# CrossmodalGroup/DynamicVectorQuantization

Measured on AMD Instinct MI355X. Metric: images/sec (256x256) DQ-VAE train step + VQ argmin GB/s, 1/2/4/8 MI355X, higher is better.
Workload: dtype bf16

## Files before the change

### dynamicvectorquantization_amd/_lib.py

```python
from __future__ import annotations

import ctypes as C
import os

HERE = os.path.dirname(os.path.abspath(__file__))
LIB_PATH = os.path.join(HERE, "libdvq_hip.so")

F32, BF16 = 0, 1
(IMPL_AUTO, IMPL_NAIVE, IMPL_MFMA, IMPL_REGSTAGE, IMPL_HALO, IMPL_WIDE, IMPL_WIDE_PIPE, IMPL_WIDE_PIPE_4WAVE, IMPL_WIDE_PIPE_192,
 IMPL_CONV_PIPE, IMPL_8PHASE) = range(11)

vp, i64, i32, f32, sz = C.c_void_p, C.c_int64, C.c_int32, C.c_float, C.c_size_t


class ConvDesc(C.Structure):
    _fields_ = [("N", i64), ("H", i64), ("W", i64), ("Cin", i64), ("OH", i64), ("OW", i64), ("Cout", i64),
                ("KH", i32), ("KW", i32), ("stride", i32), ("pad_t", i32), ("pad_l", i32), ("upsample", i32),
                ("dtype", i32), ("impl", i32)]


class DecodeLayer(C.Structure):
    _fields_ = [(n, vp) for n in ("wq", "wk", "wv", "wo", "w1", "w2", "bq", "bk", "bv", "bo", "b1", "b2", "ln1_g", "ln1_b", "ln2_g", "ln2_b",
                                  "kcache", "vcache")]


class LinPackEntry(C.Structure):
    _fields_ = [("master", vp), ("w", vp), ("wt", vp), ("out", i64), ("in_", i64), ("out_p", i64), ("tile_begin", i64),
                ("wt_ld", i64), ("bias_src", vp), ("bias_dst", vp)]


class PackEntry(C.Structure):
    _fields_ = [("master", vp), ("w", vp), ("wt", vp), ("Cout", i64), ("Cin", i64), ("taps", i64), ("Cin_p", i64),
                ("Cout_p", i64), ("begin", i64), ("dtype", i64)]


class ScalarRecord(C.Structure):
    _fields_ = [("addr", C.c_uint64 * 64), ("code", C.c_uint8 * 64)]


class JpegInfo(C.Structure):
    _fields_ = [("width", i32), ("height", i32), ("components", i32), ("restart_interval", i32), ("h_samp", i32 * 4), ("v_samp", i32 * 4),
                ("qtab_index", i32 * 4), ("supported", i32), ("reserved", i32), ("coef_count", i64)]


(JPEG_SUPPORTED, JPEG_NOT_JPEG, JPEG_MALFORMED, JPEG_PROGRESSIVE, JPEG_ARITHMETIC, JPEG_SOF_KIND, JPEG_PRECISION, JPEG_COMPONENTS,
 JPEG_SAMPLING, JPEG_COLORSPACE, JPEG_MULTISCAN) = range(11)

SCALAR_F32, SCALAR_BF16, SCALAR_F64, SCALAR_I32, SCALAR_I64, SCALAR_IMM, SCALAR_SKIP = range(7)
SCALAR_PUSH_MAX, SCALAR_COLUMNS_MAX = 64, 256


SIGNATURES = {
    "dvq_last_error": (C.c_char_p, []),
    "dvq_last_kernel": (C.c_char_p, []),
    "dvq_version": (i32, []),
    "dvq_check_device": (i32, []),
    "dvq_set_deterministic": (i32, [i32]),
    "dvq_deterministic": (i32, []),
    "dvq_unordered_launches": (C.c_longlong, []),
    "dvq_set_fp32_split": (i32, [i32]),
    "dvq_fp32_split": (i32, []),
    "dvq_probe_mfma_rate": (i32, [i32, vp, vp, vp]),
    "dvq_vq_prep_bytes": (sz, [i64, i64]),
    "dvq_vq_prepare": (i32, [vp, i64, i64, vp, vp]),
    "dvq_vq_argmin_workspace_bytes": (sz, [i64]),
    "dvq_vq_argmin": (i32, [vp, i32, vp, vp, i64, i64, i64, vp, vp, i32, vp]),
    "dvq_vq_distances": (i32, [vp, i32, vp, i64, i64, i64, vp, vp]),
    "dvq_vq_gather_loss": (i32, [vp, i32, vp, vp, vp, i64, i64, vp, vp, vp]),
    "dvq_vq_backward": (i32, [vp, vp, i32, vp, vp, vp, vp, i64, i64, vp, vp]),
    "dvq_vq_embed": (i32, [vp, vp, i64, i64, i32, vp, vp]),
    "dvq_vq_ema_stats": (i32, [vp, i32, vp, i64, i64, i64, vp, vp]),
    "dvq_vq_ema_apply": (i32, [vp, vp, f32, f32, i64, i64, vp, vp, vp, vp, vp]),
    "dvq_patch_entropy_gate": (i32, [vp, i64, i64, i64, i32, f32, vp, vp, vp]),
    "dvq_patch_entropy_gate_range": (i32, [vp, i64, i64, i64, i32, f32, f32, f32, vp, vp, vp]),
    "dvq_gn_stats": (i32, [vp, i32, i64, i64, i64, i32, vp, vp]),
    "dvq_gn_apply": (i32, [vp, i32, i64, i64, i64, i32, f32, vp, vp, vp, i32, vp, vp, vp]),
    "dvq_gn_bwd_partial_bytes": (sz, [i64, i64, i64]),
    "dvq_gn_bwd_reduce": (i32, [vp, vp, i32, i64, i64, i64, i32, vp, vp, vp, i32, vp, vp, vp, vp, vp]),
    "dvq_gn_bwd_dx": (i32, [vp, vp, i32, i64, i64, i64, i32, vp, vp, vp, i32, vp, vp, vp, vp]),
    "dvq_conv2d_fwd": (i32, [C.POINTER(ConvDesc), vp, vp, vp, vp, vp, vp, vp, i32, i32, vp]),
    "dvq_conv3x3_fused_ok": (i32, [C.POINTER(ConvDesc)]),
    "dvq_conv3x3_subpixel_ok": (i32, [C.POINTER(ConvDesc)]),
    "dvq_split_bf16_planes": (i32, [vp, vp, vp, i64, i64, i64, vp]),
    "dvq_conv3x3_x3_ok": (i32, [C.POINTER(ConvDesc), i32]),
    "dvq_conv3x3_x3_scratch_bytes": (i64, [C.POINTER(ConvDesc), i32]),
    "dvq_conv2d_fwd_x3": (i32, [C.POINTER(ConvDesc), vp, vp, vp, vp, vp, i32, vp, i64, vp]),
    "dvq_conv2d_dgrad_x3": (i32, [C.POINTER(ConvDesc), vp, vp, vp, vp, vp, i32, vp, i64, vp]),
    "dvq_conv2d_wgrad_x3_scratch_bytes": (i64, [C.POINTER(ConvDesc)]),
    "dvq_conv2d_wgrad_oihw_x3": (i32, [C.POINTER(ConvDesc), vp, vp, i64, i64, vp, vp, i32, vp, i64, vp]),
    "dvq_gn_scale_shift": (i32, [vp, vp, vp, i64, i64, i64, i32, f32, vp, vp, vp]),
    "dvq_conv2d_dgrad": (i32, [C.POINTER(ConvDesc), vp, vp, vp, vp, vp, i32, vp]),
    "dvq_set_workspace": (i32, [vp, i64]),
    "dvq_workspace_release": (i32, [vp]),
    "dvq_cmdlist_create": (i32, [vp, C.POINTER(vp)]),
    "dvq_cmdlist_replay": (i32, [vp, vp, vp]),
    "dvq_cmdlist_info": (i32, [vp, vp]),
    "dvq_cmdlist_destroy": (i32, [vp]),
    "dvq_permute_dual": (i32, [vp, vp, i64, i32, i32, i32, i64, i64, i64, i64, i64, i64, vp, vp, vp, vp, vp, vp]),
    "dvq_permute_dual_back": (i32, [vp, vp, vp, vp, i64, i64, i64, i32, i32, i64, i64, vp, vp]),
    "dvq_avgpool_slice": (i32, [vp, i32, i64, i64, i64, i64, i32, vp, i64, i64, vp]),
    "dvq_avgpool_slice_bwd": (i32, [vp, i32, i64, i64, i64, i64, i64, i64, i32, vp, vp]),
    "dvq_silu": (i32, [vp, i32, i64, vp, vp]),
    "dvq_silu_bwd": (i32, [vp, vp, i32, i64, vp, vp]),
    "dvq_relu": (i32, [vp, i32, i64, vp, vp]),
    "dvq_relu_bwd": (i32, [vp, vp, i32, i64, vp, vp]),
    "dvq_upsample_nearest2x": (i32, [vp, i32, i64, i64, i64, i64, vp, vp]),
    "dvq_upsample_nearest2x_bwd": (i32, [vp, i32, i64, i64, i64, i64, vp, vp]),
    "dvq_grain_merge": (i32, [vp, i32, vp, vp, i32, i64, i64, i64, i64, vp, vp, vp]),
    "dvq_grain_merge_bwd": (i32, [vp, vp, i32, vp, vp, i32, i64, i64, i64, i64, vp, vp, vp]),
    "dvq_affine_channels": (i32, [vp, i32, i64, i64, vp, vp, vp, vp]),
    "dvq_axpy_dev": (i32, [vp, vp, vp, i32, i64, vp, vp]),
    "dvq_maxpool2x2": (i32, [vp, i32, i64, i64, i64, i64, vp, vp]),
    "dvq_maxpool2x2_relu_bwd": (i32, [vp, vp, vp, i32, i64, i64, i64, i64, vp, vp]),
    "dvq_lpips_head": (i32, [vp, vp, vp, i32, i64, i64, i64, vp, f32, vp, vp]),
    "dvq_lpips_head_drop": (i32, [vp, vp, vp, i32, i64, i64, i64, vp, f32, vp, f32, C.c_uint64, vp]),
    "dvq_conv2d_wgrad": (i32, [C.POINTER(ConvDesc), vp, vp, i64, i64, vp, vp, i32, vp, vp]),
    "dvq_pack_weights_multi": (i32, [vp, i64, i64, vp]),
    "dvq_linear_pack_multi": (i32, [vp, i64, i64, vp]),
    "dvq_pack_weight": (i32, [vp, i64, i64, i64, i64, i64, i64, i32, vp, vp, vp]),
    "dvq_unpack_wgrad": (i32, [vp, i64, i64, i64, i64, i64, vp, vp]),
    "dvq_nchw_to_nhwc_pad": (i32, [vp, i64, i64, i64, i64, i64, i32, vp, vp]),
    "dvq_nhwc_pad_to_nchw": (i32, [vp, i32, i64, i64, i64, i64, i64, vp, vp]),
    "dvq_gemm_nt": (i32, [vp, vp, vp, i32, i64, i64, i64, i64, i64, i64, i64, i64, i64, i64, f32, vp, i32, i32, vp]),
    "dvq_gemm_tn": (i32, [vp, vp, vp, vp, i32, i64, i64, i64, i64, i64, i64, i64, i64, i64, i64, i32, vp]),
    "dvq_softmax_rows": (i32, [vp, i32, i64, i64, f32, vp, vp]),
    "dvq_softmax_rows_bwd": (i32, [vp, vp, i32, i64, i64, f32, vp, vp]),
    "dvq_transpose": (i32, [vp, i32, i64, i64, i64, vp, vp]),
    "dvq_dual_merge": (i32, [vp, vp, vp, i32, i64, i64, i64, i64, vp, vp, vp]),
    "dvq_dual_merge_bwd": (i32, [vp, vp, i32, i64, i64, i64, i64, vp, vp, vp]),
    "dvq_add": (i32, [vp, vp, i32, i64, vp, vp]),
    "dvq_add_bias_bcast": (i32, [vp, vp, i32, i64, i64, vp, vp]),
    "dvq_channel_shift_add8": (i32, [vp, vp, i32, i64, i32, vp, vp]),
    "dvq_sum_batch": (i32, [vp, i32, i64, i64, vp, vp]),
    "dvq_sumpool2x2": (i32, [vp, i32, i64, i64, i64, i64, vp, vp]),
    "dvq_cast": (i32, [vp, i32, vp, i32, i64, vp]),
    "dvq_l1_loss": (i32, [vp, vp, i64, vp, vp, vp, vp]),
    "dvq_adam": (i32, [vp, vp, vp, vp, i64, f32, f32, f32, f32, i32, vp]),
    "dvq_adamw": (i32, [vp, vp, vp, vp, i64, f32, f32, f32, f32, f32, i32, vp]),
    "dvq_layernorm_fwd": (i32, [vp, i32, i64, i64, f32, vp, vp, vp, vp, vp]),
    "dvq_layernorm_bwd": (i32, [vp, vp, i32, i64, i64, vp, vp, vp, vp, vp, vp]),
    "dvq_layernorm_bwd_res": (i32, [vp, vp, vp, i32, i64, i64, vp, vp, vp, vp, vp, vp]),
    "dvq_layernorm_bwd_res_drop": (i32, [vp, vp, vp, i32, i64, i64, vp, vp, vp, vp, vp, vp, f32, C.c_uint64, vp]),
    "dvq_gelu": (i32, [vp, i32, i64, vp, vp]),
    "dvq_gelu_bwd": (i32, [vp, vp, i32, i64, vp, vp]),
    "dvq_softmax_causal": (i32, [vp, i32, i64, i64, i64, i64, f32, vp, vp]),
    "dvq_embed_gather": (i32, [vp, i64, vp, i32, i64, i64, i64, i64, i64, i32, vp, vp]),
    "dvq_embed_scatter_add": (i32, [vp, i64, vp, i32, i64, i64, i64, i64, i64, i64, i64, vp, vp]),
    "dvq_cross_entropy": (i32, [vp, i32, i64, i64, i64, vp, i64, vp, vp, vp, vp, vp]),
    "dvq_attn_decode": (i32, [vp, vp, vp, i32, i64, i64, i64, i64, i64, f32, vp, vp]),
    "dvq_attn_causal_ok": (i32, [i32, i64, i64, i32, i32]),
    "dvq_attn_causal_scratch_bytes": (i64, [i64, i64, i32, i32, i32]),
    "dvq_attn_causal_mask_bytes": (i64, [i64, i64, i32]),
    "dvq_attn_causal_fwd": (i32, [vp, vp, vp, i64, i32, i64, i64, i32, i32, f32, f32, C.c_uint64, vp, vp, vp, vp, vp]),
    "dvq_attn_causal_bwd": (i32, [vp, vp, vp, i64, vp, vp, vp, i32, i64, i64, i32, i32, f32, f32, C.c_uint64, vp, vp, vp, vp, vp, vp]),
    "dvq_attn_full_ok": (i32, [i32, i64, i64, i32]),
    "dvq_attn_full_fwd": (i32, [vp, vp, vp, i32, i64, i64, i32, f32, vp, vp, vp, vp]),
    "dvq_attn_full_bwd": (i32, [vp, vp, vp, vp, vp, vp, i32, i64, i64, i32, f32, vp, vp, vp, vp, vp]),
    "dvq_attn_decode_dev": (i32, [vp, vp, vp, vp, vp, i32, i64, i64, i64, vp, i64, f32, vp, vp]),
    "dvq_rows_dev": (i32, [vp, vp, i32, i64, i64, i64, vp, i32, vp]),
    "dvq_decode_stack_scratch_bytes": (sz, [i64, i64, i64]),
    "dvq_decode_stack_ok": (i32, [i64, i64, i32, i64, i64]),
    "dvq_decode_stack_status": (i32, [vp, i64, i64, i64, i32, vp]),
    "dvq_decode_stack": (i32, [vp, i32, i64, i64, i32, i64, i64, vp, C.c_float, vp, vp, i32, vp, vp]),
    "dvq_dropout": (i32, [vp, i32, i64, f32, C.c_uint64, vp, vp]),
    "dvq_dropout_add": (i32, [vp, vp, i32, i64, f32, C.c_uint64, vp, vp]),
    "dvq_fill_f32": (i32, [vp, f32, i64, vp]),
    "dvq_image_desc_bytes": (sz, []),
    "dvq_image_batch_transform": (i32, [vp, vp, vp, vp, i64, i32, i32, vp, vp]),
    "dvq_jpeg_info": (i32, [vp, sz, C.POINTER(JpegInfo)]),
    "dvq_jpeg_entropy_decode": (i32, [vp, sz, vp, i64, vp]),
    "dvq_jpeg_desc_bytes": (sz, []),
    "dvq_jpeg_batch_decode": (i32, [vp, vp, i64, vp, vp, vp]),
    "dvq_adamw_dev": (i32, [vp, vp, vp, vp, i64, vp, vp]),
    "dvq_grad_sqnorm_workspace_bytes": (sz, [i64]),
    "dvq_grad_sqnorm": (i32, [vp, i64, f32, i32, vp, sz, vp, vp]),
    "dvq_adamw_clip_dev": (i32, [vp, vp, vp, vp, i64, vp, vp, vp]),
    "dvq_ema_update": (i32, [vp, vp, i64, vp, vp, vp]),
    "dvq_swap_f32": (i32, [vp, vp, i64, vp]),
    "dvq_segment_stats_workspace_bytes": (sz, [i64, i64]),
    "dvq_segment_stats_state_bytes": (sz, [i64]),
    "dvq_segment_plan_bytes": (sz, [vp, i64, i64]),
    "dvq_segment_plan_build": (i32, [vp, i64, i64, vp, sz]),
    "dvq_segment_stats": (i32, [vp, vp, i64, vp, i64, vp, sz, vp, sz, vp, i32, vp, vp]),
    "dvq_copy_f32_armed": (i32, [vp, vp, i64, vp, vp]),
    "dvq_set_f32x8": (i32, [vp, f32, f32, f32, f32, f32, f32, f32, f32, vp]),
    "dvq_sample_rows": (i32, [vp, i64, i64, vp, vp]),
    "dvq_add_uniform": (i32, [vp, i64, f32, vp, vp]),
    "dvq_sample_constrained": (i32, [vp, i32, i64, i64, i64, f32, vp, i64, i64, i64, vp, i64, i64, i64, vp, i32, f32, i32, vp, vp, vp]),
    "dvq_sample_guided": (i32, [vp, i32, i64, i64, i64, f32, f32, vp, i64, i64, i64, vp, i64, i64, i64, vp, i32, f32, i32, vp, vp, vp]),
    "dvq_label_dropout": (i32, [vp, i64, f32, i64, C.c_uint64, vp, vp]),
    "dvq_recon_metrics_workspace_bytes": (sz, [i64, i64, i64]),
    "dvq_recon_metrics": (i32, [vp, vp, i64, i64, i64, i32, vp, vp, vp, vp, sz, vp]),
    "dvq_code_histogram": (i32, [vp, vp, i64, i64, i64, i64, i64, i64, i32, vp, vp, vp, vp]),
    "dvq_token_nll": (i32, [vp, i32, i64, i64, i64, vp, i64, vp, vp, vp]),
    "dvq_nll_segment_sums": (i32, [vp, vp, i64, i64, i64, vp, vp]),
    "dvq_tokens_pack": (i32, [vp, vp, i64, i32, i32, i64, vp, vp, vp, vp, vp]),
    "dvq_tokens_unpack": (i32, [vp, vp, i64, i32, i32, i32, i64, i64, i64, i64, i64, i64, i64, i64, vp, vp, vp, vp, vp]),
    "dvq_vq_trained_prep_bytes": (sz, [i64, i64]),
    "dvq_vq_trained_prepare": (i32, [vp, i64, i64, i32, vp, vp]),
    "dvq_vq_sample_argmax": (i32, [vp, i32, vp, vp, i64, i64, i64, i32, f32, vp, vp, vp]),
    "dvq_vq_gumbel_noise": (i32, [C.c_uint64, C.c_uint64, i64, i64, vp, vp]),
    "dvq_vq_codebook_grad": (i32, [vp, i32, vp, vp, vp, vp, i64, i64, i64, vp, vp]),
    "dvq_vq_mask_ratio": (i32, [vp, i64, vp, vp]),
    "dvq_vq_rownorm": (i32, [vp, i64, i64, vp, vp, vp]),
    "dvq_vq_ortho_scratch_bytes": (sz, []),
    "dvq_vq_ortho_sumsq": (i32, [vp, i64, f32, vp, vp, vp]),
    "dvq_vq_rownorm_bwd": (i32, [vp, vp, vp, vp, f32, i64, i64, vp, vp]),
    "dvq_imagelog_workspace_bytes": (sz, [i64]),
    "dvq_grain_overlay": (i32, [vp, vp, vp, i32, i64, i64, i64, i64, i64, C.c_uint32, C.c_uint32, f32, vp, vp, sz, vp]),
    "dvq_grain_lines": (i32, [vp, vp, i32, i64, i64, i64, i64, i64, vp]),
    "dvq_image_grid_shape": (i32, [i64, i64, i64, i64, i64, C.POINTER(i64), C.POINTER(i64)]),
    "dvq_image_grid_u8": (i32, [vp, i64, i64, i64, i64, i64, i64, i32, vp, sz, vp, sz, vp]),
    "dvq_scalar_push_state_bytes": (sz, [i64]),
    "dvq_scalar_push": (i32, [C.POINTER(ScalarRecord), i32, i32, i32, vp, vp]),
    "dvq_codebook_health": (i32, [vp, i32, i64, i64, vp, vp, vp, vp]),
    "dvq_codec_tables": (i32, [vp, i32, i64, i64, i64, vp, i64, i64, i64, vp, i64, i64, i64, vp, vp, vp]),
    "dvq_codec_record": (i32, [vp, i32, i64, i64, i64, vp, i64, i64, i64, vp, i64, i64, i64, vp, vp, vp, i64, i64, vp, vp, vp]),
    "dvq_codec_encode": (i32, [vp, i64, i64, i64, vp, vp, vp, i64, vp, vp, vp]),
    "dvq_codec_decode_step": (i32, [vp, i32, i64, i64, i64, vp, i64, i64, i64, vp, i64, i64, i64, vp, vp, vp, i64, vp, vp, vp]),
}


class DvqError(RuntimeError):
    pass


_lib = None


def load():
    global _lib
    if _lib is not None:
        return _lib
    import torch
    if not os.path.exists(LIB_PATH):
        raise DvqError(
            f"{LIB_PATH} not found. Build it with `python -m dynamicvectorquantization_amd.build` "
            "(hipcc, gfx950). There is no CPU fallback for the DQ-VAE hot path.")
    lib = C.CDLL(LIB_PATH)
    for name, (res, args) in SIGNATURES.items():
# ... 17 lines not shown
```

### dynamicvectorquantization_amd/csrc/attention.hip

```cpp
#include <type_traits>

#include "attn_common.h"

namespace {

template <int HS>
struct Geo {
    static constexpr int RROW = HS * 2 + 16;
    static constexpr int CROW = 64 + 16;
    static constexpr int RTILE = 32 * RROW;
    static constexpr int CTILE = HS * CROW;
    static constexpr int NCH = HS / 64;
};

template <int HS>
__device__ __forceinline__ void gload_rows(const bf16_t* base, int64_t rowbase, int r0, int T, int C, int tid, uint4 (&reg)[HS / 64]) {
#pragma unroll
    for (int i = 0; i < HS / 64; ++i) {
        const int id = tid + 256 * i, row = id / (HS / 8), cc = id % (HS / 8);
        reg[i] = r0 + row < T ? *reinterpret_cast<const uint4*>(base + (rowbase + r0 + row) * C + cc * 8) : make_uint4(0, 0, 0, 0);
    }
}
template <int HS>
__device__ __forceinline__ void swrite_rows(char* tile, int tid, const uint4 (&reg)[HS / 64]) {
// ... 368 lines not shown
                            if constexpr (EDGE) pr = (ok && (!diag || krow <= query)) ? pr : 0.f;
                            float gr = dp[r];
                            pk[i] = pr;
                            if constexpr (MASK) {
                                const bool keep = (mword >> (8 * g + i)) & 1u;
                                gr = keep ? gr * p.inv_keep : 0.f;
                                pk[i] = keep ? pr * p.inv_keep : 0.f;
                            } else {
                                if (p.thr != 0) {
                                    const unsigned idx = (unsigned)(((int64_t)bh * T + query) * T) + (unsigned)krow;
                                    const bool keep = dvq_hash32(idx * p.rm + p.ra) >= p.thr;
                                    gr = keep ? gr * p.inv_keep : 0.f;
                                    pk[i] = keep ? pr * p.inv_keep : 0.f;
                                }
                            }
                            ds[i] = pr * (gr - dq_[i]);
                        }
                        const unsigned p0 = pack_bf16x2(pk[0], pk[1]), p1 = pack_bf16x2(pk[2], pk[3]);
                        const unsigned d0 = pack_bf16x2(ds[0], ds[1]), d1 = pack_bf16x2(ds[2], ds[3]);
                        if (gg == 0) {
                            pf.u.x = p0; pf.u.y = p1; df.u.x = d0; df.u.y = d1;
                        } else {
                            pf.u.z = p0; pf.u.w = p1; df.u.z = d0; df.u.w = d1;
                        }
                    }
#pragma unroll
                    for (int mt = 0; mt < NM; ++mt) {
                        if constexpr (DO_DV) dv[mt] = MFMA(frag_c<HS>(dtl, l31, half, mt, s2), pf.v, dv[mt]);
                        if constexpr (DO_DK) dk[mt] = MFMA(frag_c<HS>(qtl, l31, half, mt, s2), df.v, dk[mt]);
                    }
                }
            };
            if (edge) second(std::true_type{});
            else second(std::false_type{});
        }
        if (more) {
            char* nl = smem + ((qt + 1 - kt_min) & 1) * STAGE;
            swrite_rows<HS>(nl, tid, rq);
            if constexpr (DO_DK) swrite_rows<HS>(nl + G::RTILE, tid, rd);
            if constexpr (DO_DK) swrite_cols<HS>(nl + 2 * G::RTILE, tid, rqt);
            if constexpr (DO_DV) swrite_cols<HS>(nl + 2 * G::RTILE + G::CTILE, tid, rdt);
        }
        __syncthreads();
    }
    if (kok) {
        if constexpr (DO_DV) store_ct<NM>(p.dv + (rowbase + krow) * C + h * HS, dv, half, 1.f);
        if constexpr (DO_DK) store_ct<NM>(p.dk + (rowbase + krow) * C + h * HS, dk, half, p.scale);
    }
}

template <int HS>
int launch_fwd(const AttnArgsCm& p, dim3 grid, hipStream_t stream) {
    using G = Geo<HS>;
    const int lds = 2 * (G::RTILE + G::CTILE);
    dvq_ensure_dynamic_lds((const void*)attn_fwd_kernel<HS>, lds);
    attn_fwd_kernel<HS><<<grid, dim3(256), lds, stream>>>(p);
    return 0;
}

template <int HS, bool MASKED>
int launch_bwd_m(const AttnArgsCm& p, dim3 grid, hipStream_t stream) {
    using G = Geo<HS>;
    const int lds_kv = 2 * (2 * G::RTILE + 2 * G::CTILE), lds_q = 2 * (2 * G::RTILE + G::CTILE);
    dvq_ensure_dynamic_lds((const void*)attn_bwd_dq_kernel<HS, MASKED>, lds_q);
    attn_bwd_dq_kernel<HS, MASKED><<<grid, dim3(256), lds_q, stream>>>(p);
    dvq_ensure_dynamic_lds((const void*)attn_bwd_dkv_kernel<HS, 0, MASKED>, lds_kv);
    attn_bwd_dkv_kernel<HS, 0, MASKED><<<grid, dim3(256), lds_kv, stream>>>(p);
    return 0;
}
template <int HS>
int launch_bwd(const AttnArgsCm& p, dim3 grid, hipStream_t stream) {
    if (p.thr != 0 && p.mask != nullptr) return launch_bwd_m<HS, true>(p, grid, stream);
    return launch_bwd_m<HS, false>(p, grid, stream);
}

const char* attn_refusal(int dtype, int64_t B, int64_t T, int n_head, int head_dim, int64_t ld, float p_drop, int causal) {
    if (!(dtype == DVQ_BF16 && (causal ? head_dim == 64 || head_dim == 128 : head_dim == 256)))
        return "%s: bf16 with head size 64 or 128 (causal) / 256 (full attention) only (use the GEMM path otherwise)";
    if (!(causal || T % 32 == 0)) return "%s: full attention needs T %% 32 == 0";
    if (!(B > 0 && T > 0 && T % 8 == 0 && n_head > 0 && B * n_head <= 65535 && p_drop >= 0.f && p_drop < 1.f && (causal || p_drop == 0.f)))
        return "%s: bad geometry (T %% 8 == 0, B * n_head <= 65535)";
    if (!((double)B * n_head * (double)T * (double)T < 4294967296.0))
        return "%s: B * n_head * T * T must stay below 2^32 (dropout element index)";
    if (ld != (int64_t)n_head * head_dim && head_dim != 128)
        return "%s: a row pitch other than n_head * head_dim needs head size 128 (the kernels of attention2.hip)";
    if (!(ld >= (int64_t)n_head * head_dim && ld % 8 == 0 && (double)T * (double)ld * 2.0 < 4294967296.0))
        return "%s: bad pitch (at least n_head * head_dim, a multiple of 8, T * pitch * 2 below 2^32)";
    return nullptr;
}

int fill_params(AttnArgs& p, const char* who, int dtype, int64_t B, int64_t T, int n_head, int head_dim, int64_t ld, float scale, float p_drop,
                uint64_t seed, int causal = 1) {
    if (const char* why = attn_refusal(dtype, B, T, n_head, head_dim, ld, p_drop, causal)) {
        dvq_set_error(why, who);
        return DVQ_ESHAPE;
    }
    p.causal = causal;
    p.B = (int)B; p.T = (int)T; p.nh = n_head; p.ldq = (int)ld;
    p.scale = scale;
    p.inv_keep = 1.f / (1.f - p_drop);
    p.thr = (unsigned)((double)p_drop * 4294967296.0);
    dvq_dropout_seed(seed, &p.rm, &p.ra);
    return DVQ_OK;
}

int64_t dsum_bytes(int64_t B, int64_t T, int n_head) { return ((B * n_head * T * 4 + 255) / 256) * 256; }

}

extern "C" {

int dvq_attn_causal_ok(int dtype, int64_t B, int64_t T, int n_head, int head_dim) {
    return attn_refusal(dtype, B, T, n_head, head_dim, (int64_t)n_head * head_dim, 0.f, 1) == nullptr;
}
int dvq_attn_full_ok(int dtype, int64_t B, int64_t T, int C) { return attn_refusal(dtype, B, T, 1, C, C, 0.f, 0) == nullptr; }

int64_t dvq_attn_causal_scratch_bytes(int64_t B, int64_t T, int n_head, int head_dim, int backward) {
    const int64_t copy = head_dim == 64 ? B * T * n_head * head_dim * 2 : 0;
    return backward ? 3 * copy + dsum_bytes(B, T, n_head) : copy;
}

int64_t dvq_attn_causal_mask_bytes(int64_t B, int64_t T, int n_head) {
    const int64_t nt = (T + 31) / 32;
    return B * n_head * nt * nt * 16 * 8;
}

int dvq_attn_causal_fwd(const void* q, const void* k, const void* v, int64_t ldqkv, int dtype, int64_t B, int64_t T, int n_head,
                        int head_dim, float scale, float p_drop, uint64_t seed, void* out, float* lse, void* scratch, void* drop_mask,
                        dvq_stream_t stream) {
    DVQ_REQUIRE(q && k && v && out && lse, DVQ_EINVAL, "dvq_attn_causal_fwd: null pointer");
    AttnArgsCm p{};
    int rc = fill_params(p, "dvq_attn_causal_fwd", dtype, B, T, n_head, head_dim, ldqkv, scale, p_drop, seed);
    if (rc != DVQ_OK) return rc;
    DVQ_REQUIRE(scratch || dvq_attn_causal_scratch_bytes(B, T, n_head, head_dim, 0) == 0, DVQ_EINVAL, "dvq_attn_causal_fwd: null scratch");
    p.q = (const bf16_t*)q; p.k = (const bf16_t*)k; p.v = (const bf16_t*)v;
    p.out = (bf16_t*)out; p.lse = lse;
    p.mask = (unsigned long long*)drop_mask;
    if (head_dim == 128) {
        dvq_attn2_fwd(p, (hipStream_t)stream);
        DVQ_CHECK_LAUNCH("attn_causal_fwd");
        return DVQ_OK;
    }
    p.vt = (const bf16_t*)scratch;
    rc = dvq_transpose(v, dtype, B, T, n_head * head_dim, scratch, stream);
    if (rc != DVQ_OK) return rc;
    const int nqt = (int)((T + 31) / 32);
    launch_fwd<64>(p, dim3((unsigned)((nqt + 3) / 4), (unsigned)(B * n_head)), (hipStream_t)stream);
    DVQ_CHECK_LAUNCH("attn_causal_fwd");
    return DVQ_OK;
}

int dvq_attn_causal_bwd(const void* q, const void* k, const void* v, int64_t ldqkv, const void* out, const void* dout, const float* lse,
                        int dtype, int64_t B, int64_t T, int n_head, int head_dim, float scale, float p_drop, uint64_t seed, void* dq,
                        void* dk, void* dv, void* scratch, const void* drop_mask, dvq_stream_t stream) {
    DVQ_REQUIRE(q && k && v && out && dout && lse && dq && dk && dv && scratch, DVQ_EINVAL, "dvq_attn_causal_bwd: null pointer");
    AttnArgsCm p{};
    int rc = fill_params(p, "dvq_attn_causal_bwd", dtype, B, T, n_head, head_dim, ldqkv, scale, p_drop, seed);
    if (rc != DVQ_OK) return rc;
    p.q = (const bf16_t*)q; p.k = (const bf16_t*)k; p.v = (const bf16_t*)v; p.o = (const bf16_t*)out; p.dout = (const bf16_t*)dout;
    p.dq = (bf16_t*)dq; p.dk = (bf16_t*)dk; p.dv = (bf16_t*)dv;
    p.lse = const_cast<float*>(lse);
    p.mask = (unsigned long long*)const_cast<void*>(drop_mask);
    if (head_dim == 128) {
        p.dsum = (float*)scratch;
        dvq_attn2_bwd(p, (hipStream_t)stream);
        DVQ_CHECK_LAUNCH("attn_causal_bwd");
        return DVQ_OK;
    }
    const int64_t C = n_head * head_dim, elems = B * T * C;
    bf16_t* qt = (bf16_t*)scratch;
    bf16_t* kt = qt + elems;
    bf16_t* dot = kt + elems;
    p.qt = qt; p.kt = kt; p.dot = dot;
    p.dsum = reinterpret_cast<float*>(dot + elems);
    if ((rc = dvq_transpose(q, dtype, B, T, C, qt, stream)) != DVQ_OK) return rc;
    if ((rc = dvq_transpose(k, dtype, B, T, C, kt, stream)) != DVQ_OK) return rc;
    if ((rc = dvq_transpose(dout, dtype, B, T, C, dot, stream)) != DVQ_OK) return rc;
    const int nt = (int)((T + 31) / 32);
    launch_bwd<64>(p, dim3((unsigned)((nt + 3) / 4), (unsigned)(B * n_head)), (hipStream_t)stream);
    DVQ_CHECK_LAUNCH("attn_causal_bwd");
    return DVQ_OK;
}

int dvq_attn_full_fwd(const void* q, const void* k, const void* v, int dtype, int64_t B, int64_t T, int C, float scale, void* out,
                      float* lse, void* , dvq_stream_t stream) {
    DVQ_REQUIRE(q && k && v && out && lse, DVQ_EINVAL, "dvq_attn_full_fwd: null pointer");
    AttnArgs p{};
    int rc = fill_params(p, "dvq_attn_full_fwd", dtype, B, T, 1, C, C, scale, 0.f, 0, 0);
    if (rc != DVQ_OK) return rc;
    p.q = (const bf16_t*)q; p.k = (const bf16_t*)k; p.v = (const bf16_t*)v;
    p.out = (bf16_t*)out; p.lse = lse;
    dvq_attn2_fwd(p, (hipStream_t)stream);
    DVQ_CHECK_LAUNCH("attn_full_fwd");
    return DVQ_OK;
}

int dvq_attn_full_bwd(const void* q, const void* k, const void* v, const void* out, const void* dout, const float* lse, int dtype,
                      int64_t B, int64_t T, int C, float scale, void* dq, void* dk, void* dv, void* scratch, dvq_stream_t stream) {
    DVQ_REQUIRE(q && k && v && out && dout && lse && dq && dk && dv && scratch, DVQ_EINVAL, "dvq_attn_full_bwd: null pointer");
    AttnArgs p{};
    int rc = fill_params(p, "dvq_attn_full_bwd", dtype, B, T, 1, C, C, scale, 0.f, 0, 0);
    if (rc != DVQ_OK) return rc;
    p.q = (const bf16_t*)q; p.k = (const bf16_t*)k; p.v = (const bf16_t*)v; p.o = (const bf16_t*)out; p.dout = (const bf16_t*)dout;
    p.dq = (bf16_t*)dq; p.dk = (bf16_t*)dk; p.dv = (bf16_t*)dv;
    p.lse = const_cast<float*>(lse);
    p.dsum = (float*)scratch;
    dvq_attn2_bwd(p, (hipStream_t)stream);
    DVQ_CHECK_LAUNCH("attn_full_bwd");
    return DVQ_OK;
}

}
```

### dynamicvectorquantization_amd/csrc/igemm.hip

```cpp
#include "igemm.h"

using namespace igemm;

namespace {

int conv_check(const dvq_conv_desc* d, const char* who) {
    dvq_note_kernel("");
    DVQ_REQUIRE(d != nullptr, DVQ_EINVAL, "%s: null descriptor", who);
    DVQ_REQUIRE(d->N > 0 && d->H > 0 && d->W > 0 && d->Cin > 0 && d->OH > 0 && d->OW > 0 && d->Cout > 0 && d->KH > 0 &&
                    d->KW > 0 && d->stride > 0 && d->pad_t >= 0 && d->pad_l >= 0,
                DVQ_ESHAPE, "%s: non-positive dimension", who);
    DVQ_REQUIRE(d->N * d->OH * d->OW < (1ll << 31) && d->N * d->H * d->W < (1ll << 31), DVQ_ESHAPE,
                "%s: more than 2^31 pixels", who);
    DVQ_REQUIRE(d->upsample == 0 || d->upsample == 1, DVQ_EINVAL, "%s: upsample must be 0 or 1 (2: dvq_conv2d_fwd / _dgrad only)", who);
    DVQ_REQUIRE(!d->upsample || (d->H % 2 == 0 && d->W % 2 == 0), DVQ_ESHAPE, "%s: upsample needs even H, W", who);
    DVQ_REQUIRE(d->dtype == DVQ_F32 || d->dtype == DVQ_BF16, DVQ_EINVAL, "%s: bad dtype", who);
    DVQ_REQUIRE((d->OH - 1) * d->stride - d->pad_t + d->KH - 1 < d->H + d->KH && (d->OW - 1) * d->stride - d->pad_l + d->KW - 1 < d->W + d->KW,
                DVQ_ESHAPE, "%s: inconsistent output size", who);
    return DVQ_OK;
}

}

int dvq_conv3x3_halo_try(const void* x, const void* w, const float* bias, const void* residual, void* y, int64_t N,
// ... 179 lines not shown
    }
    if (sub && residual == nullptr && gn_scale_shift == nullptr && act == DVQ_ACT_NONE) {
        const bf16_t* wsub = (const bf16_t*)w + d->Cout * 9 * d->Cin;
        const int rc = dvq_conv3x3_halo_subpixel_try(x, wsub, bias, y, d->N, d->H / 2, d->W / 2, d->Cin, d->Cout, 0, out_stats, out_groups,
                                                     (hipStream_t)stream);
        if (rc != 0) return rc < 0 ? rc : DVQ_OK;
    }
    if (halo_eligible(d)) {
        const int rc = dvq_conv3x3_halo_try(x, w, bias, residual, y, d->N, d->H, d->W, d->Cin, d->Cout, 0, d->upsample,
                                            gn_scale_shift, out_stats, out_groups, act_slope_of(act), 0, 0.f,
                                            (hipStream_t)stream);
        if (rc != 0) return rc < 0 ? rc : DVQ_OK;
    }
    DVQ_REQUIRE(gn_scale_shift == nullptr && out_stats == nullptr, DVQ_ESHAPE,
                "dvq_conv2d_fwd: fused GroupNorm needs a shape accepted by dvq_conv3x3_fused_ok");
    DVQ_REQUIRE(d->impl != DVQ_IMPL_HALO, DVQ_ESHAPE, "dvq_conv2d_fwd: shape not eligible for the halo kernel");
    NtParams p = conv_nt_params(d, MODE_FWD, x, w, y);
    p.R = residual; p.bias = bias; p.bias_mode = bias ? 1 : 0;
    p.act_slope = act_slope_of(act);
    if (d->dtype == DVQ_F32) return launch_nt<float>(p, 1, d->impl, (hipStream_t)stream);
    return launch_nt<bf16_t>(p, 1, d->impl, (hipStream_t)stream);
}

int dvq_sumpool2x2(const void* in, int dtype, int64_t N, int64_t h, int64_t w, int64_t C, void* out, dvq_stream_t stream);

int dvq_conv2d_dgrad(const dvq_conv_desc* d_in, const void* dy, const void* wt, void* dx, void* ws, const void* mask, int mask_act,
                     dvq_stream_t stream) {
    dvq_note_kernel("");
    DVQ_REQUIRE(d_in != nullptr, DVQ_EINVAL, "dvq_conv2d_dgrad: null descriptor");
    dvq_conv_desc dd = *d_in;
    const dvq_conv_desc* d = &dd;
    const int sub = conv_check_up2(&dd, "dvq_conv2d_dgrad");
    if (sub < 0) return sub;
    DVQ_REQUIRE(mask == nullptr || ((mask_act == DVQ_ACT_RELU || mask_act == DVQ_ACT_LRELU) && !d->upsample), DVQ_EINVAL,
                "dvq_conv2d_dgrad: mask needs act in {relu, lrelu} and no folded upsample");
    DVQ_REQUIRE(dy && wt && dx && (!d->upsample || ws || sub), DVQ_EINVAL, "dvq_conv2d_dgrad: null pointer");
    if (sub) {
        const bf16_t* wsub = (const bf16_t*)wt + d->Cin * 9 * d->Cout;
        const int rc = dvq_conv3x3_halo_subpixel_try(dy, wsub, nullptr, dx, d->N, d->H / 2, d->W / 2, d->Cin, d->Cout, 1, nullptr, 0,
                                                     (hipStream_t)stream);
        if (rc < 0) return rc;
        DVQ_REQUIRE(rc == 1, DVQ_ESHAPE, "dvq_conv2d_dgrad: the halo kernel refused the sub-pixel form");
        return DVQ_OK;
    }
    if (d->dtype == DVQ_BF16 && d->impl == DVQ_IMPL_AUTO && d->KH == 4 && d->KW == 4 && d->stride == 2 && d->pad_t == 1 && d->pad_l == 1 &&
        d->Cin == 8 && !d->upsample && mask == nullptr && d->H == 2 * d->OH && d->W == 2 * d->OW) {
        const int rc = dvq_tconv4x4s2_thin_try(dy, wt, dx, d->N, d->OH, d->OW, d->Cout, 4, (hipStream_t)stream);
        if (rc != 0) return rc < 0 ? rc : DVQ_OK;
    }
    if (halo_eligible(d) && d->impl == DVQ_IMPL_AUTO && d->Cout == 8 && !d->upsample && mask == nullptr) {
        const int rc = dvq_conv3x3_thin_k_try(dy, wt, nullptr, dx, d->N, d->H, d->W, d->Cin, 1, 1.f, (hipStream_t)stream);
        if (rc != 0) return rc < 0 ? rc : DVQ_OK;
    }
    if (halo_eligible(d)) {
        const int rc = dvq_conv3x3_halo_try(dy, wt, nullptr, mask, d->upsample ? ws : dx, d->N, d->H, d->W, d->Cout, d->Cin, 1,
                                            0, nullptr, nullptr, 0, 1.f, mask != nullptr, act_slope_of(mask_act),
                                            (hipStream_t)stream);
        if (rc < 0) return rc;
        if (rc == 1) return d->upsample ? dvq_sumpool2x2(ws, d->dtype, d->N, d->H / 2, d->W / 2, d->Cin, dx, stream) : DVQ_OK;
    }
    DVQ_REQUIRE(d->impl != DVQ_IMPL_HALO, DVQ_ESHAPE, "dvq_conv2d_dgrad: shape not eligible for the halo kernel");
    NtParams p = conv_nt_params(d, MODE_TCONV, dy, wt, d->upsample ? ws : dx);
    p.R = mask; p.res_mask = mask != nullptr; p.mask_slope = act_slope_of(mask_act);
    int rc = d->dtype == DVQ_F32 ? launch_nt<float>(p, 1, d->impl, (hipStream_t)stream)
                                 : launch_nt<bf16_t>(p, 1, d->impl, (hipStream_t)stream);
    if (rc) return rc;
    if (d->upsample) return dvq_sumpool2x2(ws, d->dtype, d->N, d->H / 2, d->W / 2, d->Cin, dx, stream);
    return DVQ_OK;
}

int dvq_conv2d_wgrad(const dvq_conv_desc* d, const void* x, const void* dy, int64_t cin_real, int64_t cout_real, float* grad,
                     float* dbias, int ohwi, const float* gn_scale_shift, dvq_stream_t stream) {
    if (int e = conv_check(d, "dvq_conv2d_wgrad")) return e;
    DVQ_REQUIRE(x && dy && grad && cin_real > 0 && cin_real <= d->Cin && cout_real > 0 && cout_real <= d->Cout,
                DVQ_EINVAL, "dvq_conv2d_wgrad: bad arguments");
    if (halo_eligible(d)) {
        const int rc = dvq_conv3x3_halo_wgrad_try(x, dy, grad, dbias, d->N, d->H, d->W, d->Cin, d->Cout, cin_real,
                                                  cout_real, ohwi ? 0 : 1, d->upsample, gn_scale_shift, (hipStream_t)stream);
        if (rc != 0) return rc < 0 ? rc : DVQ_OK;
    }
    DVQ_REQUIRE(gn_scale_shift == nullptr, DVQ_ESHAPE, "dvq_conv2d_wgrad: fused GroupNorm needs a shape accepted by dvq_conv3x3_fused_ok");
    DVQ_REQUIRE(d->impl != DVQ_IMPL_HALO, DVQ_ESHAPE, "dvq_conv2d_wgrad: shape not eligible for the halo kernel");
    const TnParams p = conv_tn_params(d, x, dy, cin_real, cout_real, grad, dbias, ohwi);
    if (d->dtype == DVQ_F32) return launch_tn<float>(p, 1, d->impl, (hipStream_t)stream);
    return launch_tn<bf16_t>(p, 1, d->impl, (hipStream_t)stream);
}

namespace {

__global__ __launch_bounds__(256) void split_planes_kernel(const float* __restrict__ x, bf16_t* __restrict__ hi, bf16_t* __restrict__ lo,
                                                           int64_t rows, int cin, int cout) {
    const int cpr = cout >> 3;
    const int64_t total = rows * cpr;
    for (int64_t i = (int64_t)blockIdx.x * 256 + threadIdx.x; i < total; i += (int64_t)gridDim.x * 256) {
        const int64_t r = i / cpr;
        const int c0 = (int)(i - r * cpr) << 3;
        const float* src = x + r * cin + c0;
        float4 a = make_float4(0.f, 0.f, 0.f, 0.f), b = a;
        if (c0 < cin) a = *reinterpret_cast<const float4*>(src);
        if (c0 + 4 < cin) b = *reinterpret_cast<const float4*>(src + 4);
        const float v[8] = {a.x, a.y, a.z, a.w, b.x, b.y, b.z, b.w};
        uint4 h, l;
        unsigned* hp = &h.x;
        unsigned* lp = &l.x;
#pragma unroll
        for (int e = 0; e < 4; ++e) {
            const unsigned ph = pack_bf16x2(v[2 * e], v[2 * e + 1]);
            hp[e] = ph;
            lp[e] = pack_bf16x2(v[2 * e] - __uint_as_float(ph << 16), v[2 * e + 1] - __uint_as_float(ph & 0xffff0000u));
        }
        *reinterpret_cast<uint4*>(hi + r * cout + c0) = h;
        *reinterpret_cast<uint4*>(lo + r * cout + c0) = l;
    }
}

inline int64_t pad8(int64_t c) { return (c + 7) & ~(int64_t)7; }

}

int dvq_split_bf16_planes(const float* x, void* hi, void* lo, int64_t rows, int64_t cin, int64_t cout, dvq_stream_t stream) {
    DVQ_REQUIRE(x && hi && lo, DVQ_EINVAL, "dvq_split_bf16_planes: null pointer");
    DVQ_REQUIRE(rows > 0 && cin > 0 && cin % 4 == 0 && cout % 8 == 0 && cout >= cin && cout < (1 << 20), DVQ_ESHAPE,
                "dvq_split_bf16_planes: needs cin %% 4 == 0, cout %% 8 == 0, cout >= cin");
    const int64_t total = rows * (cout / 8);
    int64_t blocks = cdiv64(total, 256);
    if (blocks > 256 * 64) blocks = 256 * 64;
    split_planes_kernel<<<dim3((unsigned)blocks), dim3(256), 0, (hipStream_t)stream>>>(x, (bf16_t*)hi, (bf16_t*)lo, rows, (int)cin, (int)cout);
    DVQ_CHECK_LAUNCH("split_planes");
    return DVQ_OK;
}

int64_t dvq_conv2d_wgrad_x3_scratch_bytes(const dvq_conv_desc* d) {
    if (d == nullptr || d->dtype != DVQ_F32) return 0;
    const int64_t xrows = d->N * (d->H >> d->upsample) * (d->W >> d->upsample), yrows = d->N * d->OH * d->OW;
    return 4 * (xrows * pad8(d->Cin) + yrows * pad8(d->Cout)) + 1024;
}

int dvq_conv2d_wgrad_oihw_x3(const dvq_conv_desc* d, const void* x, const void* dy, int64_t cin_real, int64_t cout_real,
                             float* grad_oihw, float* dbias, int ohwi, void* scratch, int64_t scratch_bytes, dvq_stream_t stream) {
    if (int e = conv_check(d, "dvq_conv2d_wgrad_oihw_x3")) return e;
    DVQ_REQUIRE(d->dtype == DVQ_F32, DVQ_EINVAL, "dvq_conv2d_wgrad_oihw_x3: fp32 operands only");
    DVQ_REQUIRE(x && dy && grad_oihw && scratch && cin_real > 0 && cin_real <= d->Cin && cout_real > 0 && cout_real <= d->Cout,
                DVQ_EINVAL, "dvq_conv2d_wgrad_oihw_x3: bad arguments");
    DVQ_REQUIRE(scratch_bytes >= dvq_conv2d_wgrad_x3_scratch_bytes(d) && ((uintptr_t)scratch & 15) == 0, DVQ_EWORKSPACE,
                "dvq_conv2d_wgrad_oihw_x3: scratch too small (dvq_conv2d_wgrad_x3_scratch_bytes) or not 16-B aligned");
    const int64_t xrows = d->N * (d->H >> d->upsample) * (d->W >> d->upsample), yrows = d->N * d->OH * d->OW;
    const int64_t c8 = pad8(d->Cin), o8 = pad8(d->Cout);
    auto up256 = [](int64_t v) { return (v + 255) & ~(int64_t)255; };
    char* base = (char*)scratch;
    char* xh = base;
    char* xl = xh + up256(xrows * c8 * 2);
    char* yh = xl + up256(xrows * c8 * 2);
    char* yl = yh + up256(yrows * o8 * 2);
    if (int e = dvq_split_bf16_planes((const float*)x, xh, xl, xrows, d->Cin, c8, stream)) return e;
    if (int e = dvq_split_bf16_planes((const float*)dy, yh, yl, yrows, d->Cout, o8, stream)) return e;
    dvq_conv_desc b = *d;
    b.dtype = DVQ_BF16;
    b.Cin = c8;
    b.Cout = o8;
    if (halo_eligible(&b) && xl == xh + xrows * c8 * 2 && yl == yh + yrows * o8 * 2) {
        const int rc = dvq_conv3x3_halo_wgrad_planes_try(xh, yh, grad_oihw, dbias, d->N, d->H, d->W, c8, o8, cin_real, cout_real, ohwi ? 0 : 1,
                                                         d->upsample, (hipStream_t)stream);
        if (rc < 0) return rc;
        if (rc == 1) return DVQ_OK;
    }
    if (int e = dvq_conv2d_wgrad(&b, xl, yh, cin_real, cout_real, grad_oihw, nullptr, ohwi, nullptr, stream)) return e;
// ... 104 lines not shown
```

### dynamicvectorquantization_amd/csrc/misc.hip

```cpp
#include <stdarg.h>

#include "dvq_common.h"
#include <stdlib.h>

static thread_local char g_err[512] = "";
thread_local const char* dvq_kernel_note = "";
void dvq_set_error(const char* fmt, ...) {
    va_list ap;
    va_start(ap, fmt);
    vsnprintf(g_err, sizeof(g_err), fmt, ap);
    va_end(ap);
}

#include <atomic>
#include <mutex>
#include <vector>
void dvq_ensure_dynamic_lds(const void* kernel, int bytes) {
    static std::mutex mu;
    static std::vector<std::pair<const void*, int>> done;
    std::lock_guard<std::mutex> lock(mu);
    for (auto& e : done)
        if (e.first == kernel && e.second >= bytes) return;
    (void)hipFuncSetAttribute(kernel, hipFuncAttributeMaxDynamicSharedMemorySize, bytes);
    done.emplace_back(kernel, bytes);
// ... 215 lines not shown

template <typename T>
__global__ __launch_bounds__(256) void sum_batch_vec_kernel(const T* __restrict__ x, int64_t batch, int64_t inner8,
                                                            float* __restrict__ out, int64_t rows_per_chunk, int cvb_log2,
                                                            float* __restrict__ part) {
    __shared__ float red[256 * 8];
    const int cvb = 1 << cvb_log2, rlanes = 256 >> cvb_log2;
    const int cv = threadIdx.x & (cvb - 1), rl = threadIdx.x >> cvb_log2;
    const int64_t c8 = (int64_t)blockIdx.x * cvb + cv;
    const int64_t b0 = (int64_t)blockIdx.y * rows_per_chunk, b1 = min(batch, b0 + rows_per_chunk);
    float acc[8] = {0.f, 0.f, 0.f, 0.f, 0.f, 0.f, 0.f, 0.f};
    if (c8 < inner8) {
        for (int64_t b = b0 + rl; b < b1; b += rlanes) {
            float v[8];
            load8(x + (b * inner8 + c8) * 8, v);
#pragma unroll
            for (int j = 0; j < 8; ++j) acc[j] += v[j];
        }
    }
#pragma unroll
    for (int j = 0; j < 8; ++j) red[(rl * cvb + cv) * 8 + j] = acc[j];
    __syncthreads();
    const int ncol = cvb * 8;
    if ((int)threadIdx.x < ncol) {
        float t = 0.f;
        for (int r = 0; r < rlanes; ++r) t += red[r * ncol + threadIdx.x];
        const int64_t col = (int64_t)blockIdx.x * ncol + threadIdx.x;
        if (col < inner8 * 8) {
            if (gridDim.y == 1) out[col] += t;
            else if (part != nullptr) part[(int64_t)blockIdx.y * inner8 * 8 + col] = t;
            else atomicAdd(&out[col], t);
        }
    }
}

template <typename T>
__global__ __launch_bounds__(256) void sumpool2x2_kernel(const T* __restrict__ in, int64_t N, int64_t h, int64_t w,
                                                         int64_t C, T* __restrict__ out) {
    const int64_t cv = C / 8;
    const int64_t total = N * h * w * cv;
    for (int64_t e = (int64_t)blockIdx.x * 256 + threadIdx.x; e < total; e += (int64_t)gridDim.x * 256) {
        const int64_t c8 = e % cv, cell = e / cv;
        const int64_t xc = cell % w, yc = (cell / w) % h, n = cell / (h * w);
        float acc[8] = {0, 0, 0, 0, 0, 0, 0, 0};
#pragma unroll
        for (int dy = 0; dy < 2; ++dy)
#pragma unroll
            for (int dx = 0; dx < 2; ++dx) {
                float v[8];
                load8(in + (((n * 2 * h + 2 * yc + dy) * 2 * w) + 2 * xc + dx) * C + c8 * 8, v);
#pragma unroll
                for (int j = 0; j < 8; ++j) acc[j] += v[j];
            }
        store8(out + cell * C + c8 * 8, acc);
    }
}

template <typename TI, typename TO>
__global__ __launch_bounds__(256) void cast_kernel(const TI* __restrict__ in, TO* __restrict__ out, int64_t n) {
    for (int64_t e = (int64_t)blockIdx.x * 256 + threadIdx.x; e < n; e += (int64_t)gridDim.x * 256)
        ElemIO<TO>::store(out + e, ElemIO<TI>::load(in + e));
}

__device__ __forceinline__ float subpixel_weight(const float* m, int64_t co, int64_t ci, int cls, int t, int64_t Cin, bool ohwi) {
    const int py = cls >> 1, px = cls & 1, a = t >> 1, b = t & 1;
    const int u0 = a ? 1 + py : 0, u1 = a ? 2 : py, v0 = b ? 1 + px : 0, v1 = b ? 2 : px;
    float s = 0.f;
    for (int u = u0; u <= u1; ++u)
        for (int v = v0; v <= v1; ++v) s += master_at(m, co, ci, u * 3 + v, Cin, 9, ohwi);
    return s;
}
__device__ __forceinline__ float subpixel_w_at(const float* m, unsigned f, unsigned Cout, unsigned Cin, bool ohwi) {
    const unsigned row = f / Cin, ci = f - row * Cin, t = row & 3, r2 = row >> 2, cls = r2 / Cout, co = r2 - cls * Cout;
    return subpixel_weight(m, co, ci, (int)cls, (int)t, Cin, ohwi);
}
__device__ __forceinline__ float subpixel_wt_at(const float* m, unsigned f, unsigned Cout, unsigned Cin, bool ohwi) {
    const unsigned row = f / Cout, co = f - row * Cout, t = row & 3, cls = (row >> 2) & 3, ci = row >> 4;
    return subpixel_weight(m, co, ci, (int)cls, (int)t, Cin, ohwi);
}

template <typename T>
__global__ __launch_bounds__(256) void pack_weight_kernel(const float* __restrict__ m, int64_t Cout, int64_t Cin,
                                                          int64_t KH, int64_t KW, int64_t Cin_p, int64_t Cout_p,
                                                          T* __restrict__ w, T* __restrict__ wt, bool ohwi, bool sub) {
    const int64_t taps = KH * KW;
    const int64_t nw = w ? Cout * taps * Cin_p : 0, nwt = wt ? Cin * taps * Cout_p : 0, nsub = sub ? 16 * Cout * Cin : 0;
    for (int64_t e = (int64_t)blockIdx.x * 256 + threadIdx.x; e < nw + nwt + 2 * nsub; e += (int64_t)gridDim.x * 256) {
        if (e >= nw + nwt) {
            const int64_t f = e - nw - nwt;
            if (f < nsub) ElemIO<T>::store(w + nw + f, subpixel_w_at(m, (unsigned)f, (unsigned)Cout, (unsigned)Cin, ohwi));
            else ElemIO<T>::store(wt + nwt + f - nsub, subpixel_wt_at(m, (unsigned)(f - nsub), (unsigned)Cout, (unsigned)Cin, ohwi));
        } else if (e < nw) {
            const int64_t ci = e % Cin_p, tap = (e / Cin_p) % taps, co = e / (Cin_p * taps);
            ElemIO<T>::store(w + e, ci < Cin ? master_at(m, co, ci, tap, Cin, taps, ohwi) : 0.f);
        } else {
            const int64_t f = e - nw;
            const int64_t co = f % Cout_p, tap = (f / Cout_p) % taps, ci = f / (Cout_p * taps);
            ElemIO<T>::store(wt + f, co < Cout ? master_at(m, co, ci, tap, Cin, taps, ohwi) : 0.f);
        }
    }
}

struct PackEntry {
    const float* master;
    void* w;
    void* wt;
    int64_t Cout, Cin, taps, Cin_p, Cout_p;
    int64_t begin;
    int64_t dtype;
};

__device__ __forceinline__ float master_at(const float* m, int64_t co, int64_t ci, int64_t tap, int64_t Cin, int64_t taps, bool ohwi) {
    return ohwi ? m[(co * taps + tap) * Cin + ci] : m[(co * Cin + ci) * taps + tap];
}

__global__ __launch_bounds__(256) void pack_weights_multi_kernel(const PackEntry* __restrict__ tab, int n, int64_t total) {
    for (int64_t e = ((int64_t)blockIdx.x * 256 + threadIdx.x) * 4; e < total; e += (int64_t)gridDim.x * 1024) {
        int lo = 0, hi = n - 1;
        while (lo < hi) {
            const int mid = (lo + hi + 1) >> 1;
            if (tab[mid].begin <= e) lo = mid; else hi = mid - 1;
        }
        const PackEntry t = tab[lo];
        const unsigned f0 = (unsigned)(e - t.begin);
        const unsigned taps = (unsigned)t.taps, Cin = (unsigned)t.Cin, Cout = (unsigned)t.Cout;
        const unsigned nw = t.w ? Cout * taps * (unsigned)t.Cin_p : 0u;
        const bool ohwi = (t.dtype >> 8) & 1;
        const unsigned nwt = t.wt ? Cin * taps * (unsigned)t.Cout_p : 0u;
        float v[4];
        void* dst;
        unsigned di;
        if (((t.dtype >> 9) & 1) && f0 >= nw + nwt) {
            const unsigned f = f0 - nw - nwt, nsub = 16u * Cout * Cin;
#pragma unroll
            for (int u = 0; u < 4; ++u)
                v[u] = f < nsub ? subpixel_w_at(t.master, f + u, Cout, Cin, ohwi) : subpixel_wt_at(t.master, f - nsub + u, Cout, Cin, ohwi);
            dst = f < nsub ? t.w : t.wt;
            di = f < nsub ? nw + f : nwt + f - nsub;
        } else if (f0 < nw) {
            const unsigned cp = (unsigned)t.Cin_p, row = f0 / cp, ci = f0 - row * cp, co = row / taps, tap = row - co * taps;
#pragma unroll
            for (int u = 0; u < 4; ++u) v[u] = ci + u < Cin ? master_at(t.master, co, ci + u, tap, Cin, taps, ohwi) : 0.f;
            dst = t.w;
            di = f0;
        } else {
            const unsigned f = f0 - nw;
            const unsigned cp = (unsigned)t.Cout_p, row = f / cp, co = f - row * cp, ci = row / taps, tap = row - ci * taps;
#pragma unroll
            for (int u = 0; u < 4; ++u) v[u] = co + u < Cout ? master_at(t.master, co + u, ci, tap, Cin, taps, ohwi) : 0.f;
            dst = t.wt;
            di = f;
        }
        if ((t.dtype & 0xff) == DVQ_F32) {
            *reinterpret_cast<float4*>(reinterpret_cast<float*>(dst) + di) = make_float4(v[0], v[1], v[2], v[3]);
        } else {
            uint2 pk;
            pk.x = (unsigned)f32_to_bf16(v[0]) | ((unsigned)f32_to_bf16(v[1]) << 16);
            pk.y = (unsigned)f32_to_bf16(v[2]) | ((unsigned)f32_to_bf16(v[3]) << 16);
            *reinterpret_cast<uint2*>(reinterpret_cast<bf16_t*>(dst) + di) = pk;
        }
    }
}

struct LinPackEntry {
    const float* master;
    bf16_t* w;
    bf16_t* wt;
    int64_t out, in, out_p;
    int64_t tile_begin;
    int64_t wt_ld;
    const float* bias_src;
    float* bias_dst;
};

__global__ __launch_bounds__(256) void linear_pack_multi_kernel(const LinPackEntry* __restrict__ tab, int n) {
    __shared__ float tile[64][65];
    int lo = 0, hi = n - 1;
    while (lo < hi) {
        const int mid = (lo + hi + 1) >> 1;
        if (tab[mid].tile_begin <= (int64_t)blockIdx.x) lo = mid; else hi = mid - 1;
    }
    const LinPackEntry t = tab[lo];
    const int tj_n = (int)((t.in + 63) >> 6);
    const int ti = (int)(((int64_t)blockIdx.x - t.tile_begin) / tj_n), tj = (int)(((int64_t)blockIdx.x - t.tile_begin) - (int64_t)ti * tj_n);
    const int r0 = ti * 64, c0 = tj * 64;
    const int q = threadIdx.x & 15, rr = threadIdx.x >> 4;
    const int64_t wt_ld = t.wt_ld != 0 ? t.wt_ld : t.out_p;
    if (t.bias_dst != nullptr && tj == 0 && threadIdx.x < 64 && r0 + (int)threadIdx.x < t.out)
        t.bias_dst[r0 + threadIdx.x] = t.bias_src[r0 + threadIdx.x];
#pragma unroll
    for (int i = 0; i < 4; ++i) {
        const int r = rr + 16 * i, row = r0 + r, col = c0 + 4 * q;
        float v[4] = {0.f, 0.f, 0.f, 0.f};
        if (row < t.out) {
            if (col + 3 < t.in && (t.in & 3) == 0 && (reinterpret_cast<uintptr_t>(t.master) & 15) == 0) {
                const float4 f = *reinterpret_cast<const float4*>(t.master + (int64_t)row * t.in + col);
                v[0] = f.x; v[1] = f.y; v[2] = f.z; v[3] = f.w;
            } else {
#pragma unroll
                for (int u = 0; u < 4; ++u) v[u] = col + u < t.in ? t.master[(int64_t)row * t.in + col + u] : 0.f;
            }
        }
#pragma unroll
        for (int u = 0; u < 4; ++u) tile[r][4 * q + u] = v[u];
        if (row < t.out_p) {
            if (col + 3 < t.in && (t.in & 3) == 0) {
                uint2 pk;
                pk.x = (unsigned)f32_to_bf16(v[0]) | ((unsigned)f32_to_bf16(v[1]) << 16);
                pk.y = (unsigned)f32_to_bf16(v[2]) | ((unsigned)f32_to_bf16(v[3]) << 16);
                *reinterpret_cast<uint2*>(t.w + (int64_t)row * t.in + col) = pk;
            } else {
#pragma unroll
                for (int u = 0; u < 4; ++u)
                    if (col + u < t.in) t.w[(int64_t)row * t.in + col + u] = f32_to_bf16(v[u]);
            }
        }
    }
    __syncthreads();
#pragma unroll
    for (int i = 0; i < 4; ++i) {
        const int c = rr + 16 * i, col = c0 + c, row = r0 + 4 * q;
        if (col < t.in && row < t.out_p) {
            uint2 pk;
            pk.x = (unsigned)f32_to_bf16(tile[4 * q][c]) | ((unsigned)f32_to_bf16(tile[4 * q + 1][c]) << 16);
            pk.y = (unsigned)f32_to_bf16(tile[4 * q + 2][c]) | ((unsigned)f32_to_bf16(tile[4 * q + 3][c]) << 16);
            *reinterpret_cast<uint2*>(t.wt + (int64_t)col * wt_ld + row) = pk;
        }
    }
}

__global__ __launch_bounds__(256) void unpack_wgrad_kernel(const float* __restrict__ dw, int64_t Cout, int64_t Cin,
                                                           int64_t taps, int64_t Cin_p, float* __restrict__ g) {
    const int64_t n = Cout * Cin * taps;
    for (int64_t e = (int64_t)blockIdx.x * 256 + threadIdx.x; e < n; e += (int64_t)gridDim.x * 256) {
// ... 548 lines not shown
                                                                                                   npix, (bf16_t*)y);
    DVQ_CHECK_LAUNCH("channel_shift_add8");
    return DVQ_OK;
}

int dvq_add_bias_bcast(const void* x, const float* bias, int dtype, int64_t batch, int64_t inner, void* y,
                       dvq_stream_t stream) {
    DVQ_REQUIRE(x && bias && y && batch > 0 && inner > 0 && inner % 8 == 0, DVQ_EINVAL, "dvq_add_bias_bcast: bad arguments");
    DVQ_DISPATCH_DTYPE(dtype, T, add_bias_bcast_kernel<T><<<dim3(nblocks(batch * inner / 8, 256)), dim3(256), 0,
                                                            (hipStream_t)stream>>>((const T*)x, bias, batch, inner / 8,
                                                                                   (T*)y););
    DVQ_CHECK_LAUNCH("add_bias_bcast");
    return DVQ_OK;
}

int dvq_sum_batch(const void* x, int dtype, int64_t batch, int64_t inner, float* out, dvq_stream_t stream) {
    DVQ_REQUIRE(x && out && batch > 0 && inner > 0, DVQ_EINVAL, "dvq_sum_batch: bad arguments");
    const bool det = dvq_deterministic() != 0;
    if (inner % 8 == 0 && batch >= 64) {
        const int64_t inner8 = inner / 8;
        int lg = 2;
        while (lg < 5 && (1 << lg) < inner8) ++lg;
        const int64_t gx = cdiv64(inner8, 1 << lg);
        int64_t chunks = gx >= 512 ? 1 : cdiv64(512, gx);
        if (chunks > cdiv64(batch, 64)) chunks = cdiv64(batch, 64);
        int64_t rpc = cdiv64(batch, chunks);
        chunks = cdiv64(batch, rpc);
        if (gx <= 65535 && chunks <= 65535) {
            float* part = nullptr;
            if (chunks > 1 && det) {
                part = (float*)dvq_det_scratch((hipStream_t)stream, chunks * inner * 4);
                if (part == nullptr) { chunks = 1; rpc = batch; }
            } else if (chunks > 1) dvq_note_unordered();
            DVQ_DISPATCH_DTYPE(dtype, T, sum_batch_vec_kernel<T><<<dim3((unsigned)gx, (unsigned)chunks), dim3(256), 0, (hipStream_t)stream>>>(
                                             (const T*)x, batch, inner8, out, rpc, lg, part););
            DVQ_CHECK_LAUNCH("sum_batch");
            if (part != nullptr) return dvq_det_fold_f32(out, part, (int)chunks, inner, inner, (hipStream_t)stream);
            return DVQ_OK;
        }
    }
    const int64_t col_blocks = cdiv64(inner, 256);
    int64_t chunks = col_blocks >= 1024 ? 1 : cdiv64(1024, col_blocks);
    if (chunks > cdiv64(batch, 16)) chunks = cdiv64(batch, 16);
    if (chunks < 1) chunks = 1;
    int64_t rpc = cdiv64(batch, chunks);
    chunks = cdiv64(batch, rpc);
    float* part = nullptr;
    if (chunks > 1 && det) {
        part = (float*)dvq_det_scratch((hipStream_t)stream, chunks * inner * 4);
        if (part == nullptr) { chunks = 1; rpc = batch; }
    } else if (chunks > 1) dvq_note_unordered();
    DVQ_DISPATCH_DTYPE(dtype, T, sum_batch_kernel<T><<<dim3((unsigned)(col_blocks < 65535 ? col_blocks : 65535), (unsigned)chunks), dim3(256), 0,
                                                      (hipStream_t)stream>>>((const T*)x, batch, inner, out, rpc, part););
    DVQ_CHECK_LAUNCH("sum_batch");
    if (part != nullptr) return dvq_det_fold_f32(out, part, (int)chunks, inner, inner, (hipStream_t)stream);
    return DVQ_OK;
}

int dvq_sumpool2x2(const void* in, int dtype, int64_t N, int64_t h, int64_t w, int64_t C, void* out,
                   dvq_stream_t stream) {
    DVQ_REQUIRE(in && out && C % 8 == 0, DVQ_EINVAL, "dvq_sumpool2x2: bad arguments");
    DVQ_DISPATCH_DTYPE(dtype, T, sumpool2x2_kernel<T><<<dim3(nblocks(N * h * w * C / 8, 256)), dim3(256), 0,
                                                        (hipStream_t)stream>>>((const T*)in, N, h, w, C, (T*)out););
    DVQ_CHECK_LAUNCH("sumpool2x2");
    return DVQ_OK;
}

int dvq_cast(const void* in, int in_dtype, void* out, int out_dtype, int64_t n, dvq_stream_t stream) {
    DVQ_REQUIRE(in && out && n > 0, DVQ_EINVAL, "dvq_cast: bad arguments");
    hipStream_t s = (hipStream_t)stream;
    dim3 grid(nblocks(n, 256)), block(256);
    if (in_dtype == DVQ_F32 && out_dtype == DVQ_BF16) cast_kernel<float, bf16_t><<<grid, block, 0, s>>>((const float*)in, (bf16_t*)out, n);
    else if (in_dtype == DVQ_BF16 && out_dtype == DVQ_F32) cast_kernel<bf16_t, float><<<grid, block, 0, s>>>((const bf16_t*)in, (float*)out, n);
    else if (in_dtype == DVQ_F32 && out_dtype == DVQ_F32) cast_kernel<float, float><<<grid, block, 0, s>>>((const float*)in, (float*)out, n);
    else if (in_dtype == DVQ_BF16 && out_dtype == DVQ_BF16) cast_kernel<bf16_t, bf16_t><<<grid, block, 0, s>>>((const bf16_t*)in, (bf16_t*)out, n);
    else {
        dvq_set_error("dvq_cast: bad dtypes");
        return DVQ_EINVAL;
    }
    DVQ_CHECK_LAUNCH("cast");
    return DVQ_OK;
}

int dvq_pack_weight(const float* master, int64_t Cout, int64_t Cin, int64_t KH, int64_t KW, int64_t Cin_p,
                    int64_t Cout_p, int dtype, void* w, void* wt, dvq_stream_t stream) {
    DVQ_REQUIRE(master && (w || wt) && Cin_p >= Cin && Cout_p >= Cout, DVQ_EINVAL, "dvq_pack_weight: bad arguments");
    const bool ohwi = (dtype >> 8) & 1;
    const bool sub = (dtype >> 9) & 1;
    DVQ_REQUIRE(!sub || (w && wt && KH == 3 && KW == 3 && Cin_p == Cin && Cout_p == Cout && 16 * Cout * Cin < (1ll << 31)), DVQ_EINVAL,
                "dvq_pack_weight: sub-pixel packs need both outputs, a 3x3 kernel and unpadded channels");
    const int64_t n = Cout * KH * KW * Cin_p + Cin * KH * KW * Cout_p + (sub ? 32 * Cout * Cin : 0);
    dtype &= 0xff;
    DVQ_DISPATCH_DTYPE(dtype, T, pack_weight_kernel<T><<<dim3(nblocks(n, 256)), dim3(256), 0, (hipStream_t)stream>>>(
                                     master, Cout, Cin, KH, KW, Cin_p, Cout_p, (T*)w, (T*)wt, ohwi, sub););
    DVQ_CHECK_LAUNCH("pack_weight");
    return DVQ_OK;
}

int dvq_pack_weights_multi(const void* table_dev, int64_t n_entries, int64_t total_work, dvq_stream_t stream) {
    DVQ_REQUIRE(table_dev && n_entries > 0 && n_entries < (1 << 30) && total_work > 0, DVQ_EINVAL, "dvq_pack_weights_multi: bad arguments");
    pack_weights_multi_kernel<<<dim3(nblocks(total_work, 1024)), dim3(256), 0, (hipStream_t)stream>>>(
        (const PackEntry*)table_dev, (int)n_entries, total_work);
    DVQ_CHECK_LAUNCH("pack_weights_multi");
    return DVQ_OK;
}

int dvq_linear_pack_multi(const void* table_dev, int64_t n_entries, int64_t total_tiles, dvq_stream_t stream) {
    DVQ_REQUIRE(table_dev && n_entries > 0 && n_entries < (1 << 30) && total_tiles > 0 && total_tiles < (1ll << 31), DVQ_EINVAL,
                "dvq_linear_pack_multi: bad arguments");
    linear_pack_multi_kernel<<<dim3((unsigned)total_tiles), dim3(256), 0, (hipStream_t)stream>>>((const LinPackEntry*)table_dev, (int)n_entries);
    DVQ_CHECK_LAUNCH("linear_pack_multi");
    return DVQ_OK;
}

int dvq_unpack_wgrad(const float* dw, int64_t Cout, int64_t Cin, int64_t KH, int64_t KW, int64_t Cin_p, float* grad,
                     dvq_stream_t stream) {
    DVQ_REQUIRE(dw && grad && Cin_p >= Cin, DVQ_EINVAL, "dvq_unpack_wgrad: bad arguments");
    unpack_wgrad_kernel<<<dim3(nblocks(Cout * Cin * KH * KW, 256)), dim3(256), 0, (hipStream_t)stream>>>(
        dw, Cout, Cin, KH * KW, Cin_p, grad);
    DVQ_CHECK_LAUNCH("unpack_wgrad");
    return DVQ_OK;
}

int dvq_nchw_to_nhwc_pad(const float* in, int64_t B, int64_t C, int64_t H, int64_t W, int64_t Cp, int dtype, void* out,
                         dvq_stream_t stream) {
    DVQ_REQUIRE(in && out && Cp >= C, DVQ_EINVAL, "dvq_nchw_to_nhwc_pad: bad arguments");
    if (C <= 4 && Cp == (dtype == DVQ_F32 ? 4 : 8)) {
        DVQ_DISPATCH_DTYPE(dtype, T, nchw_to_nhwc_px_kernel<T><<<dim3(nblocks(B * H * W, 256)), dim3(256), 0,
                                                                 (hipStream_t)stream>>>(in, B, (int)C, H * W, (T*)out););
        DVQ_CHECK_LAUNCH("nchw_to_nhwc_px");
        return DVQ_OK;
    }
    DVQ_DISPATCH_DTYPE(dtype, T, nchw_to_nhwc_pad_kernel<T><<<dim3(nblocks(B * H * W * Cp, 256)), dim3(256), 0,
                                                              (hipStream_t)stream>>>(in, B, C, H * W, Cp, (T*)out););
    DVQ_CHECK_LAUNCH("nchw_to_nhwc_pad");
    return DVQ_OK;
}

int dvq_nhwc_pad_to_nchw(const void* in, int dtype, int64_t B, int64_t C, int64_t H, int64_t W, int64_t Cp, float* out,
                         dvq_stream_t stream) {
    DVQ_REQUIRE(in && out && Cp >= C, DVQ_EINVAL, "dvq_nhwc_pad_to_nchw: bad arguments");
    DVQ_DISPATCH_DTYPE(dtype, T, nhwc_pad_to_nchw_kernel<T><<<dim3(nblocks(B * C * H * W, 256)), dim3(256), 0,
                                                              (hipStream_t)stream>>>((const T*)in, B, C, H * W, Cp, out););
    DVQ_CHECK_LAUNCH("nhwc_pad_to_nchw");
    return DVQ_OK;
}

int dvq_l1_loss(const float* x, const float* xrec, int64_t n, double* loss_sum, const float* scale_dev, float* g,
                dvq_stream_t stream) {
    DVQ_REQUIRE(x && xrec && n > 0, DVQ_EINVAL, "dvq_l1_loss: bad arguments");
    unsigned nb = nblocks(n, 1024);
    double* part = nullptr;
    if (loss_sum != nullptr && nb > 1) {
        if (dvq_deterministic() != 0) {
            part = (double*)dvq_det_scratch((hipStream_t)stream, (int64_t)nb * 8);
            if (part == nullptr) nb = 1;
        } else dvq_note_unordered();
    }
    l1_loss_kernel<<<dim3(nb), dim3(256), 0, (hipStream_t)stream>>>(x, xrec, n, loss_sum, scale_dev, g, part);
    DVQ_CHECK_LAUNCH("l1_loss");
    if (part != nullptr) return dvq_det_fold_f64(loss_sum, part, (int)nb, 1, 1, (hipStream_t)stream);
    return DVQ_OK;
}

int dvq_adam(float* p, const float* g, float* m, float* v, int64_t n, float lr, float beta1, float beta2, float eps,
             int step, dvq_stream_t stream) {
    DVQ_REQUIRE(p && g && m && v && n > 0 && step >= 1, DVQ_EINVAL, "dvq_adam: bad arguments");
    const double bc1 = 1.0 - pow((double)beta1, (double)step), bc2 = 1.0 - pow((double)beta2, (double)step);
    adam_kernel<<<dim3(nblocks(n, 1024)), dim3(256), 0, (hipStream_t)stream>>>(p, g, m, v, n, (float)(lr / bc1), beta1,
                                                                             beta2, eps, (float)(1.0 / sqrt(bc2)), 1.f);
    DVQ_CHECK_LAUNCH("adam");
    return DVQ_OK;
}

int dvq_adamw(float* p, const float* g, float* m, float* v, int64_t n, float lr, float beta1, float beta2, float eps,
              float weight_decay, int step, dvq_stream_t stream) {
    DVQ_REQUIRE(p && g && m && v && n > 0 && step >= 1 && weight_decay >= 0.f, DVQ_EINVAL, "dvq_adamw: bad arguments");
    const double bc1 = 1.0 - pow((double)beta1, (double)step), bc2 = 1.0 - pow((double)beta2, (double)step);
    adam_kernel<<<dim3(nblocks(n, 1024)), dim3(256), 0, (hipStream_t)stream>>>(p, g, m, v, n, (float)(lr / bc1), beta1,
                                                                             beta2, eps, (float)(1.0 / sqrt(bc2)),
// ... 167 lines not shown
```

### dynamicvectorquantization_amd/kernels.py

```python
from __future__ import annotations

import ctypes as C

import torch

from . import _lib
from . import runtime as rt
from ._lib import ConvDesc, check

_DT = {torch.float32: _lib.F32, torch.bfloat16: _lib.BF16}


def dt(t) -> int:
    d = t if isinstance(t, torch.dtype) else t.dtype
    if d not in _DT:
        raise TypeError(f"unsupported dtype {d}; libdvq_hip computes in float32 or bfloat16")
    return _DT[d]


def vec(dtype) -> int:
    return 4 if dtype == torch.float32 else 8


def _p(t):
# ... 298 lines not shown
              "dvq_patch_entropy_gate")
    else:
        check(lib().dvq_patch_entropy_gate_range(_p(img), b, h, w, patch, float(bins[0]), float(bins[1]), float(threshold or 0.0),
                                                 _p(ent), _p(gate), _s()), "dvq_patch_entropy_gate_range")
    return ent, gate


def gn_stats(x, groups=32):
    n, c = x.shape[0], x.shape[-1]
    hw = x.numel() // (n * c)
    stats = zeros_small((n, groups, 2), torch.float64, x.device)
    check(lib().dvq_gn_stats(_p(x), dt(x), n, hw, c, groups, _p(stats), _s()), "dvq_gn_stats")
    return stats


def gn_forward(x, gamma, beta, groups=32, eps=1e-6, silu=True, stats=None):
    n, c = x.shape[0], x.shape[-1]
    hw = x.numel() // (n * c)
    if stats is None:
        stats = gn_stats(x, groups)
    y = torch.empty_like(x)
    mr = torch.empty(n, groups, 2, dtype=torch.float32, device=x.device)
    check(lib().dvq_gn_apply(_p(x), dt(x), n, hw, c, groups, eps, _p(stats), _p(gamma), _p(beta), int(silu), _p(y), _p(mr),
                             _s()), "dvq_gn_apply")
    return y, mr


def gn_scale_shift(x, gamma, beta, groups=32, eps=1e-6, stats=None):
    n, c = x.shape[0], x.shape[-1]
    hw = x.numel() // (n * c)
    if stats is None:
        stats = gn_stats(x, groups)
    ss = torch.empty(n, c, 2, dtype=torch.float32, device=x.device)
    mr = torch.empty(n, groups, 2, dtype=torch.float32, device=x.device)
    check(lib().dvq_gn_scale_shift(_p(stats), _p(gamma), _p(beta), n, hw, c, groups, eps, _p(ss), _p(mr), _s()),
          "dvq_gn_scale_shift")
    return ss, mr


def gn_backward(x, dy, mean_rstd, gamma, beta, dgamma, dbeta, groups=32, silu=True, addend=None, fixed_stats=False):
    n, c = x.shape[0], x.shape[-1]
    hw = x.numel() // (n * c)
    red = zeros_small((n, groups, 2), torch.float64, x.device)
    part = torch.empty(lib().dvq_gn_bwd_partial_bytes(n, hw, c), dtype=torch.uint8, device=x.device)
    check(lib().dvq_gn_bwd_reduce(_p(x), _p(dy), dt(x), n, hw, c, groups, _p(mean_rstd), _p(gamma), _p(beta), int(silu),
                                  _p(red), _p(dgamma), _p(dbeta), _p(part), _s()), "dvq_gn_bwd_reduce")
    if fixed_stats:
        red.zero_()
    dx = torch.empty_like(x)
    check(lib().dvq_gn_bwd_dx(_p(x), _p(dy), dt(x), n, hw, c, groups, _p(mean_rstd), _p(gamma), _p(beta), int(silu),
                              _p(red), _p(addend), _p(dx), _s()), "dvq_gn_bwd_dx")
    return dx


def conv_desc(n, h, w, cin, cout, kh, kw, stride, pad_t, pad_l, oh, ow, upsample, dtype, impl=0) -> ConvDesc:
    return ConvDesc(n, h, w, cin, oh, ow, cout, kh, kw, stride, pad_t, pad_l, int(upsample), dt(dtype), impl)


PACK_OHWI, PACK_SUBPIXEL = 256, 512


def subpixel_pack_views(wbuf, wtbuf, cout, cin):
    n9 = cout * 9 * cin
    return (wbuf[:n9].view(cout, 3, 3, cin), wtbuf[:n9].view(cin, 3, 3, cout), wbuf[n9:].view(4, cout, 4, cin),
            wtbuf[n9:].view(cin, 4, 4, cout))


def pack_weight(master_oihw, cin_p, cout_p, dtype, want_w=True, want_wt=True, subpixel=False):
    cout, cin, kh, kw = master_oihw.shape
    dev = master_oihw.device
    if subpixel:
        w = torch.empty(25 * cout * cin, dtype=dtype, device=dev)
        wt = torch.empty(25 * cout * cin, dtype=dtype, device=dev)
        check(lib().dvq_pack_weight(_p(master_oihw), cout, cin, kh, kw, cin_p, cout_p, dt(dtype) | PACK_SUBPIXEL, _p(w), _p(wt), _s()),
              "dvq_pack_weight")
        return w, wt
    w = torch.empty(cout, kh, kw, cin_p, dtype=dtype, device=dev) if want_w else None
    wt = torch.zeros(cin_p, kh, kw, cout_p, dtype=dtype, device=dev) if want_wt else None
    check(lib().dvq_pack_weight(_p(master_oihw), cout, cin, kh, kw, cin_p, cout_p, dt(dtype), _p(w), _p(wt), _s()),
          "dvq_pack_weight")
    return w, wt


def pack_weight_into(master, cin_p, cout_p, dtype, w, wt, subpixel=False):
    cout, cin, kh, kw = master.shape
    flag = dt(dtype) | (PACK_OHWI if is_ohwi(master) else 0) | (PACK_SUBPIXEL if subpixel else 0)
    check(lib().dvq_pack_weight(_praw(master), cout, cin, kh, kw, cin_p, cout_p, flag, _p(w), _p(wt), _s()),
          "dvq_pack_weight")


def unpack_wgrad(dw, grad_oihw, cin_p):
    cout, cin, kh, kw = grad_oihw.shape
    check(lib().dvq_unpack_wgrad(_p(dw), cout, cin, kh, kw, cin_p, _p(grad_oihw), _s()), "dvq_unpack_wgrad")


def conv_fused_ok(d: ConvDesc) -> bool:
    return bool(lib().dvq_conv3x3_fused_ok(C.byref(d)))


def conv_subpixel_ok(d: ConvDesc) -> bool:
    return bool(lib().dvq_conv3x3_subpixel_ok(C.byref(d)))


def _with_subpixel(d: ConvDesc) -> ConvDesc:
    d2 = ConvDesc.from_buffer_copy(d)
    d2.upsample = 2
    return d2


ACT_NONE, ACT_SWISH, ACT_LRELU, ACT_RELU = 0, 1, 2, 3


def _x3_halo(d: ConvDesc, t, dgrad: bool) -> bool:
    return (t.dtype == torch.float32 and d.KH == 3 and d.stride == 1 and rt.switch("DVQ_X3_HALO") != "0" and
            bool(lib().dvq_fp32_split()) and bool(lib().dvq_conv3x3_x3_ok(C.byref(d), int(dgrad))))


def conv2d_fwd(d: ConvDesc, x, w, bias, residual=None, gn_ss=None, out_stats=None, out_groups=0, act=ACT_NONE, subpixel=False):
    y = torch.empty(d.N, d.OH, d.OW, d.Cout, dtype=x.dtype, device=x.device)
    fl, nb = _conv_cost(d, x.element_size())
    if gn_ss is None and out_stats is None and _x3_halo(d, x, False):
        _tag(d, "fwd x3 halo" + ("+res" if residual is not None else "") + ("+act" if act != ACT_NONE else ""))
        need = int(lib().dvq_conv3x3_x3_scratch_bytes(C.byref(d), 0))
        scratch = torch.empty(need, dtype=torch.uint8, device=x.device)
        _timed("conv_x3_halo", fl, nb, lambda: check(
            lib().dvq_conv2d_fwd_x3(C.byref(d), _p(x), _p(w), _p(bias), _p(residual), _p(y), act, _p(scratch), need, _s()),
            "dvq_conv2d_fwd_x3"))
        return y
    if _shape_tags():
        _tag(d, "fwd" + ("+res" if residual is not None else "") + ("+gn" if gn_ss is not None else "") +
             ("+st" if out_stats is not None else "") + ("+act" if act != ACT_NONE else ""))
    if out_stats is not None:
        ensure_workspace(x.device)
    dc = _with_subpixel(d) if subpixel else d
    _timed_conv(fl, nb, "dvq_conv2d_fwd", lambda:
        lib().dvq_conv2d_fwd(C.byref(dc), _p(x), _p(w), _p(bias), _p(residual), _p(y), _p(gn_ss), _p(out_stats), out_groups, act, _s()))
    return y


def conv2d_dgrad(d: ConvDesc, dy, wt, mask=None, mask_act=ACT_NONE, subpixel=False):
    sh, sw = (d.H // 2, d.W // 2) if d.upsample else (d.H, d.W)
    dx = torch.empty(d.N, sh, sw, d.Cin, dtype=dy.dtype, device=dy.device)
    ws = torch.empty(d.N, d.H, d.W, d.Cin, dtype=dy.dtype, device=dy.device) if d.upsample and not subpixel else None
    fl, nb = _conv_cost(d, dy.element_size())
    if _x3_halo(d, dy, True):
        _tag(d, "dgrad x3 halo")
        need = int(lib().dvq_conv3x3_x3_scratch_bytes(C.byref(d), 1))
        scratch = torch.empty(need, dtype=torch.uint8, device=dy.device)
        _timed("conv_x3_halo", fl, nb, lambda: check(
            lib().dvq_conv2d_dgrad_x3(C.byref(d), _p(dy), _p(wt), _p(dx), _p(ws), _p(mask), mask_act, _p(scratch), need, _s()),
            "dvq_conv2d_dgrad_x3"))
        return dx
    _tag(d, "dgrad")
    dc = _with_subpixel(d) if subpixel else d
    _timed_conv(fl, nb, "dvq_conv2d_dgrad", lambda:
        lib().dvq_conv2d_dgrad(C.byref(dc), _p(dy), _p(wt), _p(dx), _p(ws), _p(mask), mask_act, _s()))
    return dx


_workspace = {}
WORKSPACE_BYTES = 8 * (80 << 20)


def workspace_release(stream):
    if _workspace:
        lib().dvq_workspace_release(C.c_void_p(int(stream.cuda_stream)))


def copy_kernel_(dst, src):
    return torch.mul(src, 1, out=dst)


class CmdList:

    def __init__(self, graph):
        self.graph = graph
        h = C.c_void_p()
        check(lib().dvq_cmdlist_create(C.c_void_p(int(graph.raw_cuda_graph())), C.byref(h)), "dvq_cmdlist_create")
        self.handle = h
        info = (C.c_int64 * 4)()
        check(lib().dvq_cmdlist_info(h, info), "dvq_cmdlist_info")
        self.kernels, self.side_kernels, self.waits = int(info[0]), int(info[1]), int(info[2])
        self.other, self.side_open = int(info[3]) & 0xffffffff, bool(int(info[3]) >> 32)

    def replay(self, main, side):
        check(lib().dvq_cmdlist_replay(self.handle, C.c_void_p(int(main.cuda_stream)), C.c_void_p(int(side.cuda_stream))),
              "dvq_cmdlist_replay")

    def __del__(self):
        try:
            if self.handle:
                lib().dvq_cmdlist_destroy(self.handle)
                self.handle = None
        except Exception:
            pass
        self.graph = None


def ensure_workspace(device):
    device = torch.device(device)
    if _workspace.get("dev") != device:
        buf = torch.empty(WORKSPACE_BYTES, dtype=torch.uint8, device=device)
        check(lib().dvq_set_workspace(buf.data_ptr(), buf.numel()), "dvq_set_workspace")
        _workspace.update(dev=device, buf=buf)


def _wgrad_x3_planes() -> bool:
    return rt.switch("DVQ_X3_WGRAD_PLANES") != "0"


def split_bf16_planes(x2d, cout=None):
    rows, c = x2d.shape
    cout = c if cout is None else cout
    hi = torch.empty(rows, cout, dtype=torch.bfloat16, device=x2d.device)
    lo = torch.empty_like(hi)
    check(lib().dvq_split_bf16_planes(_p(x2d), _p(hi), _p(lo), rows, c, cout, _s()), "dvq_split_bf16_planes")
    return hi, lo


def conv2d_wgrad_oihw(d: ConvDesc, x, dy, cin_real, cout_real, grad_oihw, db=None, gn_ss=None):
    fl, nb = _conv_cost(d, x.element_size())
    ensure_workspace(x.device)
    if gn_ss is None and _wgrad_x3_planes() and x.dtype == torch.float32 and d.impl == 0 and bool(lib().dvq_fp32_split()):
        _tag(d, "wgrad x3 planes")
        need = int(lib().dvq_conv2d_wgrad_x3_scratch_bytes(C.byref(d)))
        scratch = torch.empty(need, dtype=torch.uint8, device=x.device)
        _timed("conv_wgrad_x3_planes", fl, nb, lambda: check(
            lib().dvq_conv2d_wgrad_oihw_x3(C.byref(d), _p(x), _p(dy), cin_real, cout_real, _praw(grad_oihw), _p(db),
                                           int(is_ohwi(grad_oihw)), _p(scratch), need, _s()), "dvq_conv2d_wgrad_oihw_x3"))
        return
    _tag(d, "wgrad")
    _timed_conv(fl, nb, "dvq_conv2d_wgrad", lambda:
        lib().dvq_conv2d_wgrad(C.byref(d), _p(x), _p(dy), cin_real, cout_real, _praw(grad_oihw), _p(db),
                               int(is_ohwi(grad_oihw)), _p(gn_ss), _s()))


def set_deterministic(on: bool):
    check(lib().dvq_set_deterministic(int(bool(on))), "dvq_set_deterministic")
    _det[0] = bool(on)


def deterministic() -> bool:
    _det[0] = bool(lib().dvq_deterministic())
    return _det[0]


def unordered_launches() -> int:
    return int(lib().dvq_unordered_launches())


def pack_weights_multi(table_dev, n_entries, total_work):
    check(lib().dvq_pack_weights_multi(_p(table_dev), n_entries, total_work, _s()), "dvq_pack_weights_multi")


def linear_pack_multi(table_dev, n_entries, total_tiles):
    check(lib().dvq_linear_pack_multi(_p(table_dev), n_entries, total_tiles, _s()), "dvq_linear_pack_multi")


_arena = {"buf": None, "off": 0}


def arena_reset(device=None, nbytes=8 << 20):
    a = _arena
    if a["buf"] is None or (device is not None and a["buf"].device != torch.device(device)):
        a["buf"] = torch.zeros(nbytes, dtype=torch.uint8, device=device or "cuda")
    else:
        a["buf"].zero_()
    a["off"] = 0


def zeros_small(shape, dtype, device):
    a = _arena
    n = 1
    for s_ in shape:
        n *= int(s_)
    nb = (n * torch.empty((), dtype=dtype).element_size() + 255) // 256 * 256
    if a["buf"] is None or a["buf"].device != torch.device(device) or a["off"] + nb > a["buf"].numel():
        return torch.zeros(shape, dtype=dtype, device=device)
    out = a["buf"][a["off"]:a["off"] + nb].view(dtype)[:n].view(shape)
    a["off"] += nb
    return out


def nchw_to_nhwc_pad(img, cp, dtype):
    b, c, h, w = img.shape
    out = torch.empty(b, h, w, cp, dtype=dtype, device=img.device)
    check(lib().dvq_nchw_to_nhwc_pad(_p(img), b, c, h, w, cp, dt(dtype), _p(out), _s()), "dvq_nchw_to_nhwc_pad")
    return out


def nhwc_pad_to_nchw(x, c):
    b, h, w, cp = x.shape
    out = torch.empty(b, c, h, w, dtype=torch.float32, device=x.device)
    check(lib().dvq_nhwc_pad_to_nchw(_p(x), dt(x), b, c, h, w, cp, _p(out), _s()), "dvq_nhwc_pad_to_nchw")
    return out


def probe_mfma_rate(random_operands=True):
    tf, mhz = C.c_float(0.0), C.c_float(0.0)
    check(lib().dvq_probe_mfma_rate(int(bool(random_operands)), C.byref(tf), C.byref(mhz), _s()), "dvq_probe_mfma_rate")
    return float(tf.value), float(mhz.value)


def gemm_nt(a, b, m, n, k, lda, ldb, ldc, batch=1, sa=0, sb=0, sc=0, alpha=1.0, bias=None, bias_mode=0, out=None,
            impl=0):
    if out is None:
        out = torch.empty(batch * m * ldc if sc == 0 else batch * sc, dtype=a.dtype, device=a.device)
    es = a.element_size()
    _timed("gemm_nt", 2 * batch * m * n * k, es * batch * (m * k + n * k + m * n), lambda: check(
        lib().dvq_gemm_nt(_p(a), _p(b), _p(out), dt(a), m, n, k, lda, ldb, ldc, batch, sa, sb, sc, alpha, _p(bias),
                          bias_mode, impl, _s()), "dvq_gemm_nt"))
    return out


def gemm_tn(a, b, mred, i, j, lda, ldb, ldc, batch=1, sa=0, sb=0, sc=0, out=None, impl=0, colsum=None):
    if out is None:
        out = torch.zeros(batch * (sc if sc else i * ldc), dtype=torch.float32, device=a.device)
    es = a.element_size()
    if a.is_cuda and es == 2 and mred >= 1024 and i >= 256 and j >= 256:
# ... 276 lines not shown

def nll_segment_sums(nll, rank, b, tp, split):
    if nll.numel() != b * tp or rank.numel() != b * tp:
        raise _lib.DvqError(f"nll_segment_sums: {nll.numel()} / {rank.numel()} rows for [{b}, {tp}]")
    out = torch.empty(b, 2, 4, dtype=torch.float64, device=nll.device)
    check(lib().dvq_nll_segment_sums(_p(nll), _p(rank), b, tp, split, _p(out), _s()), "dvq_nll_segment_sums")
    return out


def dropout_add(x, a, p, seed):
    y = torch.empty_like(x)
    check(lib().dvq_dropout_add(_p(x), _p(a), dt(x), x.numel(), float(p), int(seed) & 0xFFFFFFFFFFFFFFFF, _p(y), _s()), "dvq_dropout_add")
    return y


def dropout(x, p, seed):
    y = torch.empty_like(x)
    check(lib().dvq_dropout(_p(x), dt(x), x.numel(), float(p), int(seed) & 0xFFFFFFFFFFFFFFFF, _p(y), _s()), "dvq_dropout")
    return y


def attn_causal_ok(x, n_head, b, t):
    c = x.shape[-1]
    return (x.dtype in _DT and c % n_head == 0 and rt.switch("DVQ_NO_FUSED_ATTN") != "1" and
            bool(lib().dvq_attn_causal_ok(dt(x), b, t, n_head, c // n_head)))


def _attn_scratch(q, b, t, n_head, backward):
    nbytes = lib().dvq_attn_causal_scratch_bytes(b, t, n_head, q.shape[-1] // n_head, int(backward))
    return torch.empty(nbytes, dtype=torch.uint8, device=q.device) if nbytes else None


def _attn_pitch(a, b, c):
    s = a.stride()
    if len(s) == 2 and s[1] == 1 and b.stride() == s and c.stride() == s and a.shape == b.shape == c.shape:
        return s[0]
    if a.is_contiguous() and b.is_contiguous() and c.is_contiguous():
        return a.shape[-1]
    raise _lib.DvqError("attention operands must be contiguous, or 2-d column blocks that share one row pitch")


def attn_causal_drop_mask(q, b, t, n_head):
    return torch.empty(lib().dvq_attn_causal_mask_bytes(b, t, n_head) // 8, dtype=torch.int64, device=q.device)


def attn_causal_fwd(q, k, v, b, t, n_head, scale, p_drop=0.0, seed=0, drop_mask=None):
    ld = _attn_pitch(q, k, v)
    out = torch.empty(q.shape, dtype=q.dtype, device=q.device)
    lse = torch.empty(b, n_head, t, dtype=torch.float32, device=q.device)
    scratch = _attn_scratch(q, b, t, n_head, False)
    c = q.shape[-1]
    _timed("attn_causal_fwd", 2 * b * t * t * c, 4 * q.numel() * q.element_size(), lambda: check(
        lib().dvq_attn_causal_fwd(_praw(q), _praw(k), _praw(v), ld, dt(q), b, t, n_head, c // n_head, float(scale), float(p_drop),
                                  int(seed) & 0xFFFFFFFFFFFFFFFF, _p(out), _p(lse), _p(scratch), _p(drop_mask), _s()),
        "dvq_attn_causal_fwd"))
    return out, lse


def attn_causal_bwd(q, k, v, out, dout, lse, b, t, n_head, scale, p_drop=0.0, seed=0, drop_mask=None, grads=None):
    ld = _attn_pitch(q, k, v)
    if grads is None:
        if ld != q.shape[-1]:
            raise _lib.DvqError("attn_causal_bwd: q, k, v with a row pitch need grads laid out like them")
        grads = tuple(torch.empty_like(q) for _ in range(3))
    if _attn_pitch(*grads) != ld or grads[0].shape != q.shape:
        raise _lib.DvqError("attn_causal_bwd: grads must share the shape and row pitch of q, k, v")
    dq, dk, dv = grads
    scratch = _attn_scratch(q, b, t, n_head, True)
    c = q.shape[-1]
    _timed("attn_causal_bwd", 5 * b * t * t * c, 8 * q.numel() * q.element_size(), lambda: check(
        lib().dvq_attn_causal_bwd(_praw(q), _praw(k), _praw(v), ld, _p(out), _p(dout), _p(lse), dt(q), b, t, n_head, c // n_head,
                                  float(scale), float(p_drop), int(seed) & 0xFFFFFFFFFFFFFFFF, _praw(dq), _praw(dk), _praw(dv),
                                  _p(scratch), _p(drop_mask), _s()),
        "dvq_attn_causal_bwd"))
    return dq, dk, dv


def attn_full_ok(q, t):
    return (q.dtype in _DT and rt.switch("DVQ_NO_FUSED_ATTNBLOCK") != "1" and
            bool(lib().dvq_attn_full_ok(dt(q), q.shape[0] // max(1, t), t, q.shape[-1])))


def attn_full_fwd(q, k, v, b, t, scale):
    c = q.shape[-1]
    out = torch.empty_like(q)
    lse = torch.empty(b, t, dtype=torch.float32, device=q.device)
    scratch = _attn_scratch(q, b, t, 1, False)
    _timed("attn_full_fwd", 4 * b * t * t * c, 4 * q.numel() * q.element_size(), lambda: check(
        lib().dvq_attn_full_fwd(_p(q), _p(k), _p(v), dt(q), b, t, c, float(scale), _p(out), _p(lse), _p(scratch), _s()),
        "dvq_attn_full_fwd"))
    return out, lse


def attn_full_bwd(q, k, v, out, dout, lse, b, t, scale):
    c = q.shape[-1]
    dq, dk, dv = torch.empty_like(q), torch.empty_like(q), torch.empty_like(q)
    scratch = _attn_scratch(q, b, t, 1, True)
    _timed("attn_full_bwd", 10 * b * t * t * c, 8 * q.numel() * q.element_size(), lambda: check(
        lib().dvq_attn_full_bwd(_p(q), _p(k), _p(v), _p(out), _p(dout), _p(lse), dt(q), b, t, c, float(scale), _p(dq), _p(dk), _p(dv),
                                _p(scratch), _s()), "dvq_attn_full_bwd"))
    return dq, dk, dv


def decode_stack_scratch(b, c, f, device):
    return torch.zeros(lib().dvq_decode_stack_scratch_bytes(b, c, f), dtype=torch.uint8, device=device)


def decode_stack_ok(b, c, n_head, f, tmax) -> bool:
    return bool(lib().dvq_decode_stack_ok(b, c, n_head, f, tmax))


def decode_stack_status(scratch, b, c, f, reset=True):
    check(lib().dvq_decode_stack_status(_p(scratch), b, c, f, int(reset), _s()), "dvq_decode_stack_status")


def decode_stack(table_dev, n_layers, x, n_head, f, tmax, t_dev, eps, scratch, n_workgroups=0, table_host=None):
    b, c = x.shape
    host = None if table_host is None else C.cast(table_host, C.c_void_p)
    check(lib().dvq_decode_stack(_p(table_dev), n_layers, b, c, n_head, f, tmax, _p(t_dev), float(eps), _p(x), _p(scratch),
                                 int(n_workgroups), host, _s()), "dvq_decode_stack")
    return x


def attn_decode_dev(q, k_new, v_new, kcache, vcache, n_head, t_dev, scale):
    b, c = q.shape
    out = torch.empty_like(q)
    check(lib().dvq_attn_decode_dev(_p(q), _p(k_new), _p(v_new), _p(kcache), _p(vcache), dt(q), b, n_head, c // n_head, _p(t_dev),
                                    kcache.shape[1], scale, _p(out), _s()), "dvq_attn_decode_dev")
    return out


def rows_dev(x, hidden, t_dev, store):
    b, c = x.shape
    check(lib().dvq_rows_dev(_p(x), _p(hidden), dt(x), b, c, hidden.shape[1], _p(t_dev), int(store), _s()), "dvq_rows_dev")
    return x


def adamw_step(p, g, m, v, lr, beta1, beta2, eps, weight_decay, step):
    check(lib().dvq_adamw(_p(p), _p(g), _p(m), _p(v), p.numel(), lr, beta1, beta2, eps, weight_decay, step, _s()), "dvq_adamw")


def adamw_dev(p, g, m, v, hyper):
    check(lib().dvq_adamw_dev(_p(p), _p(g), _p(m), _p(v), p.numel(), _p(hyper), _s()), "dvq_adamw_dev")


GRAD_SQNORM_CHUNK = 32768


def grad_sqnorm_workspace_bytes(n) -> int:
    return int(lib().dvq_grad_sqnorm_workspace_bytes(int(n)))


def grad_stats_block(device):
    return torch.tensor([0, 0, 0x3F800000, 1, 0, 0, 0, 0], dtype=torch.int32, device=device)


def grad_sqnorm(g, workspace, gstat, clip=0.0, skip_nonfinite=False):
    assert g.dtype == torch.float32 and gstat.dtype == torch.int32 and gstat.numel() == 8
    check(lib().dvq_grad_sqnorm(_p(g), g.numel(), float(clip), int(bool(skip_nonfinite)), _p(workspace),
                                workspace.numel() * workspace.element_size(), _p(gstat), _s()), "dvq_grad_sqnorm")
    return gstat


def read_grad_stats(gstat) -> dict:
    h = gstat.cpu()
    return {"norm": float(h.view(torch.float64)[0]), "coef": float(h.view(torch.float32)[2]), "finite": bool(int(h[3])),
            "skipped": int(h[4])}


def adamw_clip_dev(p, g, m, v, hyper, gstat):
    check(lib().dvq_adamw_clip_dev(_p(p), _p(g), _p(m), _p(v), p.numel(), _p(hyper), _p(gstat), _s()), "dvq_adamw_clip_dev")


def ema_update(e, p, rec, gstat=None):
    assert e.dtype == torch.float32 and p.dtype == torch.float32 and rec.dtype == torch.float32 and e.numel() == p.numel()
    assert e.is_contiguous() and p.is_contiguous() and rec.numel() >= 1
    check(lib().dvq_ema_update(_p(e), _p(p), e.numel(), _p(rec), _p(gstat) if gstat is not None else None, _s()), "dvq_ema_update")
    return e


def swap_f32(a, b):
    assert a.dtype == torch.float32 and b.dtype == torch.float32 and a.numel() == b.numel()
    assert a.is_contiguous() and b.is_contiguous()
# ... 406 lines not shown
```

### dynamicvectorquantization_amd/layers.py

```python
from __future__ import annotations

import math

import torch
import torch.nn as nn

from . import kernels as K
from . import runtime as rt


class Tape:

    def __init__(self):
        self.s = {}
        self.c = {}

    def child(self, name: str) -> "Tape":
        t = self.c.get(name)
        if t is None:
            t = self.c[name] = Tape()
        return t


def _child(tape, name):
# ... 455 lines not shown
        k, s = self.kernel_size, self.stride
        if self.asym_pad:
            pt = pl = 0
            oh, ow = (h + 1 - k) // s + 1, (w + 1 - k) // s + 1
        else:
            pt = pl = self.padding
            oh, ow = (h + 2 * self.padding - k) // s + 1, (w + 2 * self.padding - k) // s + 1
        cin_p, cout_p = self._padded(x.dtype)
        assert x.shape[-1] == cin_p, f"expected {cin_p} (padded) input channels, got {x.shape[-1]}"
        return K.conv_desc(n, h, w, cin_p, cout_p, k, k, s, pt, pl, oh, ow, self.upsample, x.dtype, rt.impl())

    def _subpixel(self, d, dtype) -> bool:
        ent = self._packs.get(dtype)
        return bool(self.upsample and ent is not None and ent["sub"] and K.conv_subpixel_ok(d))

    def fused_ok(self, x) -> bool:
        return x.dtype == torch.bfloat16 and self.kernel_size == 3 and K.conv_fused_ok(self._desc(x))

    def fwd(self, x, tape, residual=None, gn_ss=None, want_stats=False, act=K.ACT_NONE):
        w, _, bias = self.packed(x.dtype)
        d = self._desc(x)
        if act != K.ACT_NONE:
            y = K.conv2d_fwd(d, x, w, bias, act=act)
            if tape is not None:
                tape.s.update(x=x, d=d, gn_ss=None)
            return y
        stats = None
        if want_stats and self.out_channels % 32 == 0 and 128 % (self.out_channels // 32) == 0 and self.fused_ok(x):
            stats = K.zeros_small((d.N, 32, 2), torch.float64, x.device)
        y = K.conv2d_fwd(d, x, w, bias, residual, gn_ss=gn_ss, out_stats=stats, out_groups=32 if stats is not None else 0,
                         subpixel=self._subpixel(d, x.dtype))
        if stats is not None:
            y._gn_stats = stats
        if tape is not None:
            tape.s.update(x=x, d=d, gn_ss=gn_ss)
        return y

    def bwd(self, dy, tape, need_dx=True, need_dw=True, mask=None, mask_act=K.ACT_NONE):
        x, d = tape.s["x"], tape.s["d"]
        side = need_dw and need_dx and rt.side_wgrad_enabled()
        dx = None
        if side:
            _, wt, _ = self.packed(x.dtype)
            dx = K.conv2d_dgrad(d, dy, wt, mask=mask, mask_act=mask_act, subpixel=self._subpixel(d, x.dtype))
        if need_dw:
            db = _grad_buf(self.bias) if self.bias is not None else None
            gw, gss = _grad_buf(self.weight), tape.s.get("gn_ss")
            if side:
                rt.run_on_side(lambda: K.conv2d_wgrad_oihw(d, x, dy, self.in_channels, self.out_channels, gw, db, gn_ss=gss), x, dy)
            else:
                K.conv2d_wgrad_oihw(d, x, dy, self.in_channels, self.out_channels, gw, db, gn_ss=gss)
        if not need_dx:
            return None
        if dx is not None:
            return dx
        _, wt, _ = self.packed(x.dtype)
        return K.conv2d_dgrad(d, dy, wt, mask=mask, mask_act=mask_act, subpixel=self._subpixel(d, x.dtype))


def conv1x1_bwd_accumulate(conv, dy, tape, acc):
    x, d = tape.s["x"], tape.s["d"]
    ok = (conv.kernel_size == 1 and conv.stride == 1 and conv.padding == 0 and not conv.upsample and not conv.asym_pad and
          dy.dtype == torch.bfloat16 and rt.impl() == 0 and acc is not None and d.Cin == conv.in_channels and d.Cout == conv.out_channels)
    if not ok:
        dx = conv.bwd(dy, tape)
        return dx if acc is None else K.add(dx, acc)
    _, wt, _ = conv.packed(x.dtype)
    dt_ = K.conv_desc(d.N, d.H, d.W, d.Cout, d.Cin, 1, 1, 1, 0, 0, d.H, d.W, False, dy.dtype, d.impl)
    dx = K.conv2d_fwd(dt_, dy, wt, None, acc)
    db = _grad_buf(conv.bias) if conv.bias is not None else None
    gw = _grad_buf(conv.weight)
    if rt.side_wgrad_enabled():
        rt.run_on_side(lambda: K.conv2d_wgrad_oihw(d, x, dy, conv.in_channels, conv.out_channels, gw, db), x, dy)
    else:
        K.conv2d_wgrad_oihw(d, x, dy, conv.in_channels, conv.out_channels, gw, db)
    return dx


class _PackRegistry:

    def __init__(self):
        self.items = {}
        self.tables = {}
        self.retired = []

    def register(self, mod, dtype):
        import weakref
        key = (dtype, mod.weight.device)
        self.items.setdefault(key, []).append(weakref.ref(mod))
        for k in [k for k in self.tables if k[:2] == key]:
            self.retired.append(self.tables.pop(k))

    def repack(self, dtype, device, group=0):
        import ctypes
        from ._lib import PackEntry
        key = (dtype, device)
        mods = [m for m in (r() for r in self.items.get(key, [])) if m is not None and dtype in m._packs and
                getattr(m.weight, "_dvq_group", 0) == group]
        key = (dtype, device, group)
        live = [m for m in mods if m._packs[dtype]["master"] == m.weight.data_ptr() and m._packs[dtype]["w"].device == device]
        if len(live) < 2:
            return
        sig = tuple((m.weight.data_ptr(), m._packs[dtype]["w"].data_ptr(), m.weight.stride()) for m in live)
        tab = self.tables.get(key)
        if tab is None or tab["sig"] != sig:
            arr = (PackEntry * len(live))()
            begin = 0
            for i, m in enumerate(live):
                e = m._packs[dtype]
                k2 = m.kernel_size * m.kernel_size
                arr[i] = PackEntry(m.weight.data_ptr(), e["w"].data_ptr(), e["wt"].data_ptr(), m.out_channels, m.in_channels,
                                   k2, e["cin_p"], e["cout_p"], begin, K.dt(dtype) | (K.PACK_OHWI if K.is_ohwi(m.weight) else 0) |
                                   (K.PACK_SUBPIXEL if e["sub"] else 0))
                begin += m.out_channels * k2 * e["cin_p"] + m.in_channels * k2 * e["cout_p"]
                if e["sub"]:
                    begin += 32 * m.out_channels * m.in_channels
            raw = torch.frombuffer(bytearray(bytes(arr)), dtype=torch.uint8).to(device)
            tab = {"sig": sig, "table": raw, "n": len(live), "total": begin}
            if key in self.tables:
                self.retired.append(self.tables[key])
            self.tables[key] = tab
        K.pack_weights_multi(tab["table"], tab["n"], tab["total"])
        for m in live:
            m._packs[dtype]["epoch"] = m._pack_key()


PACKS = _PackRegistry()


class Upsample(HipModule):

    def __init__(self, in_channels, with_conv):
        super().__init__()
        self.with_conv = with_conv
        if with_conv:
            self.conv = Conv2d(in_channels, in_channels, 3, stride=1, padding=1, upsample=True)

    def fwd(self, x, tape):
        if not self.with_conv:
            return K.upsample_nearest2x(x)
        return self.conv.fwd(x, _child(tape, "conv"), want_stats=True)

    def bwd(self, dy, tape):
        if not self.with_conv:
            return K.upsample_nearest2x_bwd(dy)
        return self.conv.bwd(dy, tape.child("conv"))


class Downsample(HipModule):

    def __init__(self, in_channels, with_conv):
        super().__init__()
        self.with_conv = with_conv
        if with_conv:
            self.conv = Conv2d(in_channels, in_channels, 3, stride=2, padding=0, asym_pad=True)

    def fwd(self, x, tape):
        if not self.with_conv:
            n, h, w, c = x.shape
            y = torch.empty(n, h // 2, w // 2, c, dtype=x.dtype, device=x.device)
            K.avgpool_slice(x[:, : 2 * (h // 2), : 2 * (w // 2)].contiguous() if (h | w) & 1 else x, 2, y, 0)
            if tape is not None:
                tape.s["in_hw"] = (h, w)
            return y
        return self.conv.fwd(x, _child(tape, "conv"))

    def bwd(self, dy, tape):
        if not self.with_conv:
            dx = K.avgpool_slice_bwd(dy, 0, dy.shape[-1], 2)
            h, w = tape.s["in_hw"]
            if (h | w) & 1:
                dx = torch.nn.functional.pad(dx, (0, 0, 0, w - dx.shape[2], 0, h - dx.shape[1]))
            return dx
        return self.conv.bwd(dy, tape.child("conv"))


def norm_swish_conv(norm, conv, x, tape, nname, cname, residual=None):
    if (rt.fuse_gn_prologue() or tape is None) and conv.fused_ok(x):
        ss = norm.prep(x, _child(tape, nname))
        return conv.fwd(x, _child(tape, cname), residual=residual, gn_ss=ss, want_stats=True)
    a = norm.fwd(x, _child(tape, nname), silu=True)
    return conv.fwd(a, _child(tape, cname), residual=residual, want_stats=True)


class ResnetBlock(HipModule):

    def __init__(self, *, in_channels, out_channels=None, conv_shortcut=False, dropout=0.0, temb_channels=512):
        super().__init__()
        out_channels = in_channels if out_channels is None else out_channels
        if temb_channels > 0:
            raise NotImplementedError("temb_channels > 0 is unused by the DQ-VAE (temb is None)")
        self.dropout = nn.Dropout(dropout)
        self.in_channels, self.out_channels = in_channels, out_channels
        self.use_conv_shortcut = conv_shortcut
        self.norm1 = Normalize(in_channels)
        self.conv1 = Conv2d(in_channels, out_channels, 3, 1, 1)
        self.norm2 = Normalize(out_channels)
        self.conv2 = Conv2d(out_channels, out_channels, 3, 1, 1)
        if in_channels != out_channels:
            if conv_shortcut:
                self.conv_shortcut = Conv2d(in_channels, out_channels, 3, 1, 1)
            else:
                self.nin_shortcut = Conv2d(in_channels, out_channels, 1, 1, 0)

    def _shortcut(self):
        return self.conv_shortcut if self.use_conv_shortcut else self.nin_shortcut

    def forward(self, x, temb=None, **kw):
        assert temb is None
        return super().forward(x, **kw)

    def fwd(self, x, tape, temb=None):
        h1 = norm_swish_conv(self.norm1, self.conv1, x, tape, "norm1", "conv1")
        sc = self._shortcut().fwd(x, _child(tape, "nin")) if self.in_channels != self.out_channels else x
        if self.training and self.dropout.p > 0.0:
            a = self.norm2.fwd(h1, _child(tape, "norm2"), silu=True)
            seed = rt.next_dropout_seed()
            if tape is not None:
                tape.s["drop"] = (float(self.dropout.p), seed)
            a = K.dropout(a, float(self.dropout.p), seed)
            return self.conv2.fwd(a, _child(tape, "conv2"), residual=sc, want_stats=True)
        return norm_swish_conv(self.norm2, self.conv2, h1, tape, "norm2", "conv2", residual=sc)

    def bwd(self, dy, tape):
        d = self.conv2.bwd(dy, tape.child("conv2"))
        if "drop" in tape.s:
            d = K.dropout(d, *tape.s["drop"])
        d = self.norm2.bwd(d, tape.child("norm2"))
        d = self.conv1.bwd(d, tape.child("conv1"))
        sc = self._shortcut().bwd(dy, tape.child("nin")) if self.in_channels != self.out_channels else dy
        return self.norm1.bwd(d, tape.child("norm1"), addend=sc)


class AttnBlock(HipModule):

    def __init__(self, in_channels):
        super().__init__()
        self.in_channels = in_channels
        self.norm = Normalize(in_channels)
        self.q = Conv2d(in_channels, in_channels, 1)
        self.k = Conv2d(in_channels, in_channels, 1)
        self.v = Conv2d(in_channels, in_channels, 1)
        self.proj_out = Conv2d(in_channels, in_channels, 1)

    def fwd(self, x, tape):
        b, h, w, c = x.shape
        n = h * w
        hn = self.norm.fwd(x, _child(tape, "norm"), silu=False)
        q = self.q.fwd(hn, _child(tape, "q"))
        k = self.k.fwd(hn, _child(tape, "k"))
        v = self.v.fwd(hn, _child(tape, "v"))
        impl = rt.impl()
        if impl == 0 and K.attn_full_ok(q.view(b * n, c), n):
            o, lse = K.attn_full_fwd(q.view(b * n, c), k.view(b * n, c), v.view(b * n, c), b, n, float(int(c) ** (-0.5)))
            y = self.proj_out.fwd(o.view(b, h, w, c), _child(tape, "proj"), residual=x)
            if tape is not None:
                tape.s.update(q=q, k=k, v=v, o=o, lse=lse, p=None, shape=(b, h, w, c))
            return y
        s = K.gemm_nt(q, k, n, n, c, c, c, n, batch=b, sa=n * c, sb=n * c, sc=n * n, impl=impl)
        p = K.softmax_rows(s, b * n, n, float(int(c) ** (-0.5)))
        vt = K.transpose(v, b, n, c)
        o = K.gemm_nt(p, vt, n, c, n, n, n, c, batch=b, sa=n * n, sb=c * n, sc=n * c, impl=impl)
        o = o.view(b, h, w, c)
        y = self.proj_out.fwd(o, _child(tape, "proj"), residual=x)
        if tape is not None:
            tape.s.update(q=q, k=k, v=v, p=p, shape=(b, h, w, c))
        return y

    def bwd(self, dy, tape):
        st = tape.s
        b, h, w, c = st["shape"]
        n = h * w
        q, k, v, p = st["q"], st["k"], st["v"], st["p"]
        impl = rt.impl()
        do = self.proj_out.bwd(dy, tape.child("proj"))
        if p is None:
            dq, dk, dv = K.attn_full_bwd(q.view(b * n, c), k.view(b * n, c), v.view(b * n, c), st["o"], do.view(b * n, c), st["lse"],
                                         b, n, float(int(c) ** (-0.5)))
            dh = self.q.bwd(dq.view(b, h, w, c), tape.child("q"))
            dh = conv1x1_bwd_accumulate(self.k, dk.view(b, h, w, c), tape.child("k"), dh)
            dh = conv1x1_bwd_accumulate(self.v, dv.view(b, h, w, c), tape.child("v"), dh)
            return self.norm.bwd(dh, tape.child("norm"), addend=dy)
        dp = K.gemm_nt(do, v, n, n, c, c, c, n, batch=b, sa=n * c, sb=n * c, sc=n * n, impl=impl)
        dv32 = K.gemm_tn(p, do, n, n, c, n, c, c, batch=b, sa=n * n, sb=n * c, sc=n * c, impl=impl)
        ds = K.softmax_rows_bwd(p, dp, b * n, n, float(int(c) ** (-0.5)))
        kt = K.transpose(k, b, n, c)
        dq = K.gemm_nt(ds, kt, n, c, n, n, n, c, batch=b, sa=n * n, sb=c * n, sc=n * c, impl=impl)
        dk32 = K.gemm_tn(ds, q, n, n, c, n, c, c, batch=b, sa=n * n, sb=n * c, sc=n * c, impl=impl)
        dt_ = q.dtype
        dq = dq.view(b, h, w, c)
        dk = K.cast(dk32.view(b, h, w, c), dt_)
        dv = K.cast(dv32.view(b, h, w, c), dt_)
        dh = self.q.bwd(dq, tape.child("q"))
        dh = conv1x1_bwd_accumulate(self.k, dk, tape.child("k"), dh)
        dh = conv1x1_bwd_accumulate(self.v, dv, tape.child("v"), dh)
        return self.norm.bwd(dh, tape.child("norm"), addend=dy)
```

### dynamicvectorquantization_amd/runtime.py

```python
from __future__ import annotations

import contextlib
import os

import torch

from . import _lib

_compute_dtype = torch.float32
_weights_epoch = 0
IMPL_CHOICES = (_lib.IMPL_AUTO, _lib.IMPL_NAIVE, _lib.IMPL_MFMA, _lib.IMPL_REGSTAGE, _lib.IMPL_HALO, _lib.IMPL_CONV_PIPE)
_impl = _lib.IMPL_AUTO


SWITCHES = {
    "DVQ_FUSE_GN": ("0", "1: GroupNorm+swish inside the consuming 3x3 conv on taped forwards too"),
    "DVQ_X3_HALO": ("1", "0: fp32x3 3x3 forward / input gradient on the fp32 kernel that splits at every fragment read"),
    "DVQ_X3_WGRAD_PLANES": ("1", "0: fp32x3 weight gradients on the fp32 kernel that splits at every fragment read"),
    "DVQ_NO_FUSED_ATTN": ("0", "1: causal attention as per-head GEMMs + softmax instead of the fused kernels"),
    "DVQ_NO_FUSED_ATTNBLOCK": ("0", "1: AttnBlock on GEMMs + softmax (stores the [B,N,N] probabilities)"),
    "DVQ_QKV_FUSED": ("1", "0: key / query / value as three Linear layers instead of one GEMM"),
    "DVQ_FUSE_DROP_BWD": ("1", "0: stand-alone dropout passes in the StackGPT backward"),
    "DVQ_GEN_SIDE": ("1", "0: generator loss with the PatchGAN branch on the main stream"),
    "DVQ_LOSS_PREFETCH": ("1", "0: target-only loss work inside the loss call instead of beside the autoencoder's forward"),
    "DVQ_SIDE_WGRAD": ("1", "0: weight gradients on the main stream"),
    "DVQ_STEP_GRAPH": ("1", "0: every training step eager, nothing recorded"),
    "DVQ_DECODE_GRAPH": ("1", "0: single-row sampler steps eager, nothing recorded"),
    "DVQ_DECODE_STACK": ("1", "0: a sampler token step as per-kernel launches instead of the persistent kernel"),
    "DVQ_DECODE_WGS": ("0", "n: workgroups of the persistent token-step kernel (0: the library chooses)"),
    "DVQ_PROFILE_SHAPES": ("0", "1: the profiler splits the conv families by call geometry"),
    "DVQ_GRAPH_DEBUG": ("0", "1: print the library calls of every recorded segment, synchronise after every replayed item"),
    "DVQ_GRAPH_BREAK_EVERY": ("0", "n: with DVQ_GRAPH_DEBUG=1, cut a recorded segment every n library calls"),
    "DVQ_FORCE_DP": ("0", "1: the data-parallel path in a one-rank group"),
    "DVQ_DP_CHECK_EVERY": ("0", "k: assert that the replicas are equal every k steps"),
    "DVQ_DP_NO_HOOK": ("0", "1: no all-reduce launch from inside the backward"),
    "DVQ_DP_NOOP_COLLECTIVES": ("0", "1: exchange points without the RCCL calls"),
}


def switch(name: str) -> str:
    return os.environ.get(name, SWITCHES[name][0])


def force_dp() -> bool:
    return switch("DVQ_FORCE_DP") == "1"


def compute_dtype() -> torch.dtype:
    return _compute_dtype


_fp32_split = None


def fp32_split() -> bool:
    from . import _lib
    return bool(_lib.load().dvq_fp32_split())


def set_fp32_split(on):
    global _fp32_split
    from . import _lib
    _fp32_split = None if on is None else bool(on)
    if on is not None:
        _lib.check(_lib.load().dvq_set_fp32_split(int(bool(on))), "dvq_set_fp32_split")


def set_compute_dtype(dtype):
    global _compute_dtype
    if isinstance(dtype, str):
        if dtype in ("fp32x3", "float32x3"):
            set_fp32_split(True)
            dtype = torch.float32
        else:
            if dtype in ("fp32", "float32") and _fp32_split:
                set_fp32_split(False)
            dtype = {"fp32": torch.float32, "float32": torch.float32, "bf16": torch.bfloat16, "bfloat16": torch.bfloat16}[dtype]
    assert dtype in (torch.float32, torch.bfloat16)
    _compute_dtype = dtype


@contextlib.contextmanager
def compute_dtype_ctx(dtype):
    global _fp32_split
    old, old_flag = _compute_dtype, _fp32_split
    old_lib = fp32_split() if isinstance(dtype, str) and dtype.startswith(("fp32", "float32")) else None
    set_compute_dtype(dtype)
    try:
        yield
    finally:
        set_compute_dtype(old)
        if old_lib is not None and fp32_split() != old_lib:
            set_fp32_split(old_lib)
        _fp32_split = old_flag


def weights_epoch() -> int:
    return _weights_epoch


def bump_weights_epoch():
    global _weights_epoch
    _weights_epoch += 1

# ... 288 lines not shown
```

### include/dvq_hip.h

```cpp
#ifndef DVQ_HIP_H
#define DVQ_HIP_H

#include <stddef.h>
#include <stdint.h>

#ifdef __cplusplus
extern "C" {
#endif

typedef void* dvq_stream_t;
typedef void* dvq_cmdlist_t;

enum { DVQ_F32 = 0, DVQ_BF16 = 1 };
enum { DVQ_OK = 0, DVQ_EINVAL = -1, DVQ_ESHAPE = -2, DVQ_EARCH = -3, DVQ_ELAUNCH = -4, DVQ_EWORKSPACE = -5 };

const char* dvq_last_error(void);
const char* dvq_last_kernel(void);
int dvq_version(void);
int dvq_check_device(void);
int dvq_set_deterministic(int on);
int dvq_deterministic(void);
long long dvq_unordered_launches(void);
int dvq_set_fp32_split(int on);
int dvq_fp32_split(void);
// ... 11 lines not shown

int dvq_vq_gather_loss(const void* x, int dtype, const float* codebook, const int64_t* idx, const float* mask,
                       int64_t N, int64_t D, void* x_q, double* loss_sum, dvq_stream_t stream);
int dvq_vq_backward(const void* g_xq, const void* x, int dtype, const float* codebook, const int64_t* idx,
                    const float* mask, const float* coef_dev, int64_t N, int64_t D, void* dx, dvq_stream_t stream);
int dvq_vq_embed(const float* codebook, const int64_t* idx, int64_t N, int64_t D, int out_dtype, void* out,
                 dvq_stream_t stream);

int dvq_vq_ema_stats(const void* x, int dtype, const int64_t* idx, int64_t N, int64_t K, int64_t D, float* stats,
                     dvq_stream_t stream);
int dvq_vq_ema_apply(const float* stats, const float* restart_rows, float decay, float eps, int64_t K, int64_t D,
                     float* cluster_size_ema, float* embed_ema, float* weight, float* scratch_sum,
                     dvq_stream_t stream);

int dvq_patch_entropy_gate(const float* img, int64_t B, int64_t H, int64_t W, int patch, float threshold,
                           float* entropy, int64_t* gate, dvq_stream_t stream);
int dvq_patch_entropy_gate_range(const float* img, int64_t B, int64_t H, int64_t W, int patch, float bin_lo, float bin_hi,
                                 float threshold, float* entropy, int64_t* gate, dvq_stream_t stream);

int dvq_gn_stats(const void* x, int dtype, int64_t N, int64_t HW, int64_t C, int G, double* stats,
                 dvq_stream_t stream);
int dvq_gn_apply(const void* x, int dtype, int64_t N, int64_t HW, int64_t C, int G, float eps, const double* stats,
                 const float* gamma, const float* beta, int silu, void* y, float* mean_rstd, dvq_stream_t stream);
size_t dvq_gn_bwd_partial_bytes(int64_t N, int64_t HW, int64_t C);
int dvq_gn_bwd_reduce(const void* x, const void* dy, int dtype, int64_t N, int64_t HW, int64_t C, int G,
                      const float* mean_rstd, const float* gamma, const float* beta, int silu, double* red,
                      float* dgamma, float* dbeta, float* partials, dvq_stream_t stream);
int dvq_gn_bwd_dx(const void* x, const void* dy, int dtype, int64_t N, int64_t HW, int64_t C, int G,
                  const float* mean_rstd, const float* gamma, const float* beta, int silu, const double* red,
                  const void* addend, void* dx, dvq_stream_t stream);

enum {
    DVQ_IMPL_AUTO = 0,
    DVQ_IMPL_NAIVE = 1,
    DVQ_IMPL_MFMA = 2,
    DVQ_IMPL_REGSTAGE = 3,
    DVQ_IMPL_HALO = 4,
    DVQ_IMPL_WIDE = 5,
    DVQ_IMPL_WIDE_PIPE = 6,
    DVQ_IMPL_WIDE_PIPE_4WAVE = 7,
    DVQ_IMPL_WIDE_PIPE_192 = 8,
    DVQ_IMPL_CONV_PIPE = 9,
    DVQ_IMPL_8PHASE = 10
};

typedef struct dvq_conv_desc {
    int64_t N;
    int64_t H, W;
    int64_t Cin;
    int64_t OH, OW;
    int64_t Cout;
    int32_t KH, KW;
    int32_t stride;
    int32_t pad_t, pad_l;
    int32_t upsample;
    int32_t dtype;
    int32_t impl;
} dvq_conv_desc;

enum { DVQ_ACT_NONE = 0, DVQ_ACT_SWISH = 1, DVQ_ACT_LRELU = 2, DVQ_ACT_RELU = 3 };

int dvq_conv3x3_fused_ok(const dvq_conv_desc* d);
int dvq_conv3x3_subpixel_ok(const dvq_conv_desc* d);
int dvq_conv2d_fwd(const dvq_conv_desc* d, const void* x, const void* w, const float* bias, const void* residual, void* y,
                   const float* gn_scale_shift, double* out_stats, int out_groups, int act, dvq_stream_t stream);
int dvq_split_bf16_planes(const float* x, void* hi, void* lo, int64_t rows, int64_t cin, int64_t cout, dvq_stream_t stream);
int64_t dvq_conv2d_wgrad_x3_scratch_bytes(const dvq_conv_desc* d);
int dvq_conv2d_wgrad_oihw_x3(const dvq_conv_desc* d, const void* x, const void* dy, int64_t cin_real, int64_t cout_real,
                             float* grad_oihw, float* dbias, int ohwi, void* scratch, int64_t scratch_bytes, dvq_stream_t stream);
int dvq_conv3x3_x3_ok(const dvq_conv_desc* d, int dgrad);
int64_t dvq_conv3x3_x3_scratch_bytes(const dvq_conv_desc* d, int dgrad);
int dvq_conv2d_fwd_x3(const dvq_conv_desc* d, const void* x, const void* w, const float* bias, const void* residual, void* y, int act,
                      void* scratch, int64_t scratch_bytes, dvq_stream_t stream);
int dvq_conv2d_dgrad_x3(const dvq_conv_desc* d, const void* dy, const void* wt, void* dx, void* ws, const void* mask, int mask_act,
                        void* scratch, int64_t scratch_bytes, dvq_stream_t stream);
int dvq_gn_scale_shift(const double* stats, const float* gamma, const float* beta, int64_t N, int64_t HW, int64_t C, int G,
                       float eps, float* scale_shift, float* mean_rstd, dvq_stream_t stream);

int dvq_conv2d_dgrad(const dvq_conv_desc* d, const void* dy, const void* wt, void* dx, void* ws, const void* mask, int mask_act,
                     dvq_stream_t stream);

int dvq_conv2d_wgrad(const dvq_conv_desc* d, const void* x, const void* dy, int64_t cin_real, int64_t cout_real, float* grad,
                     float* dbias, int ohwi, const float* gn_scale_shift, dvq_stream_t stream);

int dvq_pack_weights_multi(const void* table_dev, int64_t n_entries, int64_t total_work, dvq_stream_t stream);
int dvq_linear_pack_multi(const void* table_dev, int64_t n_entries, int64_t total_tiles, dvq_stream_t stream);

int dvq_pack_weight(const float* master, int64_t Cout, int64_t Cin, int64_t KH, int64_t KW, int64_t Cin_p,
                    int64_t Cout_p, int dtype, void* w, void* wt, dvq_stream_t stream);
int dvq_unpack_wgrad(const float* dw, int64_t Cout, int64_t Cin, int64_t KH, int64_t KW, int64_t Cin_p, float* grad,
                     dvq_stream_t stream);
int dvq_nchw_to_nhwc_pad(const float* in, int64_t B, int64_t C, int64_t H, int64_t W, int64_t Cp, int dtype, void* out,
                         dvq_stream_t stream);
int dvq_nhwc_pad_to_nchw(const void* in, int dtype, int64_t B, int64_t C, int64_t H, int64_t W, int64_t Cp, float* out,
                         dvq_stream_t stream);

int dvq_gemm_nt(const void* A, const void* B, void* C, int dtype, int64_t M, int64_t N, int64_t K, int64_t lda,
                int64_t ldb, int64_t ldc, int64_t batch, int64_t sA, int64_t sB, int64_t sC, float alpha,
                const float* bias, int bias_mode, int impl, dvq_stream_t stream);
int dvq_gemm_tn(const void* A, const void* B, float* C, float* colsum, int dtype, int64_t Mred, int64_t I, int64_t J, int64_t lda,
                int64_t ldb, int64_t ldc, int64_t batch, int64_t sA, int64_t sB, int64_t sC, int impl, dvq_stream_t stream);

int dvq_set_workspace(void* ptr, int64_t bytes);
int dvq_workspace_release(dvq_stream_t stream);

int dvq_cmdlist_create(void* hip_graph, dvq_cmdlist_t* out);
int dvq_cmdlist_replay(dvq_cmdlist_t list, dvq_stream_t main_stream, dvq_stream_t side_stream);
int dvq_cmdlist_info(dvq_cmdlist_t list, int64_t* info4);
int dvq_cmdlist_destroy(dvq_cmdlist_t list);

int dvq_affine_channels(const void* x, int dtype, int64_t n, int64_t C, const float* a, const float* b, void* y,
                        dvq_stream_t stream);
int dvq_axpy_dev(const void* a, const void* b, const float* scale_dev, int dtype, int64_t n, void* y, dvq_stream_t stream);
int dvq_maxpool2x2(const void* x, int dtype, int64_t N, int64_t h, int64_t w, int64_t C, void* y, dvq_stream_t stream);
int dvq_maxpool2x2_relu_bwd(const void* a, const void* dpool, const void* dtap, int dtype, int64_t N, int64_t h, int64_t w,
                            int64_t C, void* dz, dvq_stream_t stream);
int dvq_lpips_head(const void* f0, const void* f1, const float* lin, int dtype, int64_t N, int64_t HW, int64_t C, float* val,
                   float gscale, void* df1, dvq_stream_t stream);
int dvq_lpips_head_drop(const void* f0, const void* f1, const float* lin, int dtype, int64_t N, int64_t HW, int64_t C, float* val,
                        float gscale, void* df1, float p_drop, uint64_t seed, dvq_stream_t stream);

int dvq_avgpool_slice(const void* x, int dtype, int64_t N, int64_t h, int64_t w, int64_t C, int k, void* y, int64_t ldy,
                      int64_t coff, dvq_stream_t stream);
int dvq_avgpool_slice_bwd(const void* dy, int dtype, int64_t ldy, int64_t coff, int64_t N, int64_t h, int64_t w, int64_t C,
                          int k, void* dx, dvq_stream_t stream);
int dvq_silu(const void* x, int dtype, int64_t n, void* y, dvq_stream_t stream);
int dvq_silu_bwd(const void* x, const void* dy, int dtype, int64_t n, void* dx, dvq_stream_t stream);
int dvq_relu(const void* x, int dtype, int64_t n, void* y, dvq_stream_t stream);
int dvq_relu_bwd(const void* x, const void* dy, int dtype, int64_t n, void* dx, dvq_stream_t stream);
int dvq_upsample_nearest2x(const void* x, int dtype, int64_t N, int64_t h, int64_t w, int64_t C, void* y, dvq_stream_t stream);
int dvq_upsample_nearest2x_bwd(const void* dy, int dtype, int64_t N, int64_t h, int64_t w, int64_t C, void* dx, dvq_stream_t stream);
int dvq_grain_merge(const void* const* heads, int S, const int64_t* idx, const float* scale, int dtype, int64_t N, int64_t hc,
                    int64_t wc, int64_t C, void* out, float* mask, dvq_stream_t stream);
int dvq_grain_merge_bwd(const void* g_out, const void* const* heads, int S, const int64_t* idx, const float* scale, int dtype,
                        int64_t N, int64_t hc, int64_t wc, int64_t C, void* const* dheads, float* dscale, dvq_stream_t stream);

int dvq_permute_dual(const int64_t* indices, const int64_t* grain, int64_t B, int hw1, int hw2, int order, int64_t content_pad,
                     int64_t content_eos, int64_t cpos_pad, int64_t cpos_eos, int64_t fpos_pad, int64_t fpos_eos,
                     int64_t* coarse_content, int64_t* coarse_position, int64_t* fine_content, int64_t* fine_position,
                     int* counts, dvq_stream_t stream);
int dvq_permute_dual_back(const int64_t* coarse_content, const int64_t* fine_content, const int64_t* coarse_position,
                          const int64_t* fine_position, int64_t B, int64_t Lc, int64_t Lf, int hw1, int hw2, int64_t cpos_eos,
                          int64_t fpos_eos, int64_t* out, dvq_stream_t stream);

int dvq_softmax_rows(const void* s, int dtype, int64_t rows, int64_t L, float scale, void* p, dvq_stream_t stream);
int dvq_softmax_rows_bwd(const void* p, const void* dp, int dtype, int64_t rows, int64_t L, float scale, void* ds,
                         dvq_stream_t stream);
int dvq_transpose(const void* in, int dtype, int64_t batch, int64_t R, int64_t C, void* out, dvq_stream_t stream);

int dvq_dual_merge(const void* h_fine, const void* h_coarse, const int64_t* grain, int dtype, int64_t B, int64_t h,
                   int64_t w, int64_t C, void* h_dual, float* mask, dvq_stream_t stream);
int dvq_dual_merge_bwd(const void* g_dual, const int64_t* grain, int dtype, int64_t B, int64_t h, int64_t w,
                       int64_t C, void* g_fine, void* g_coarse, dvq_stream_t stream);
int dvq_add(const void* a, const void* b, int dtype, int64_t n, void* y, dvq_stream_t stream);
int dvq_add_bias_bcast(const void* x, const float* bias, int dtype, int64_t batch, int64_t inner, void* y,
                       dvq_stream_t stream);
int dvq_channel_shift_add8(const void* a, const void* b, int dtype, int64_t npix, int shift, void* y, dvq_stream_t stream);
int dvq_sum_batch(const void* x, int dtype, int64_t batch, int64_t inner, float* out, dvq_stream_t stream);
int dvq_sumpool2x2(const void* in, int dtype, int64_t N, int64_t h, int64_t w, int64_t C, void* out,
                   dvq_stream_t stream);
int dvq_cast(const void* in, int in_dtype, void* out, int out_dtype, int64_t n, dvq_stream_t stream);
int dvq_l1_loss(const float* x, const float* xrec, int64_t n, double* loss_sum, const float* scale_dev, float* g,
                dvq_stream_t stream);
int dvq_adam(float* p, const float* g, float* m, float* v, int64_t n, float lr, float beta1, float beta2, float eps,
             int step, dvq_stream_t stream);
int dvq_adamw(float* p, const float* g, float* m, float* v, int64_t n, float lr, float beta1, float beta2, float eps,
              float weight_decay, int step, dvq_stream_t stream);

int dvq_layernorm_fwd(const void* x, int dtype, int64_t rows, int64_t C, float eps, const float* gamma, const float* beta, void* y,
                      float* mean_rstd, dvq_stream_t stream);
int dvq_layernorm_bwd(const void* x, const void* dy, int dtype, int64_t rows, int64_t C, const float* mean_rstd, const float* gamma,
                      void* dx, float* dgamma, float* dbeta, dvq_stream_t stream);
int dvq_layernorm_bwd_res(const void* x, const void* dy, const void* dres, int dtype, int64_t rows, int64_t C, const float* mean_rstd,
                          const float* gamma, void* dx, float* dgamma, float* dbeta, dvq_stream_t stream);
int dvq_layernorm_bwd_res_drop(const void* x, const void* dy, const void* dres, int dtype, int64_t rows, int64_t C, const float* mean_rstd,
                               const float* gamma, void* dx, float* dgamma, float* dbeta, void* dx_drop, float p_drop, uint64_t seed,
                               dvq_stream_t stream);
int dvq_gelu(const void* x, int dtype, int64_t n, void* y, dvq_stream_t stream);
int dvq_gelu_bwd(const void* x, const void* dy, int dtype, int64_t n, void* dx, dvq_stream_t stream);
int dvq_softmax_causal(const void* s, int dtype, int64_t rows, int64_t L, int64_t Tq, int64_t offset, float scale, void* p,
                       dvq_stream_t stream);
int dvq_embed_gather(const int64_t* idx, int64_t idx_bstride, const float* table, int dtype, int64_t B, int64_t len, int64_t Ttot,
                     int64_t t0, int64_t C, int accumulate, void* out, dvq_stream_t stream);
int dvq_embed_scatter_add(const int64_t* idx, int64_t idx_bstride, const void* dout, int dtype, int64_t B, int64_t len, int64_t Ttot,
                          int64_t t0, int64_t C, int64_t padding_idx, int64_t V, float* dtable, dvq_stream_t stream);
int dvq_cross_entropy(const void* logits, int dtype, int64_t rows, int64_t V, int64_t ldl, const int64_t* target, int64_t ignore_index,
                      float* loss_sum, float* count, const float* gscale_dev, void* dlogits, dvq_stream_t stream);
int dvq_sample_constrained(const void* logits, int dtype, int64_t B, int64_t V, int64_t ldl, float temperature,
                           const int64_t* forbid_idx, int64_t n_forbid, int64_t forbid_ld, int64_t forbid_from,
                           const int64_t* forbid_codes4, int64_t keep_code, int64_t late_forbid_code, int64_t pad_code,
                           const float* finished, int top_k, float top_p, int sample, uint64_t* state, int64_t* out,
                           dvq_stream_t stream);
int dvq_sample_guided(const void* logits, int dtype, int64_t B, int64_t V, int64_t ldl, float guidance, float temperature,
                      const int64_t* forbid_idx, int64_t n_forbid, int64_t forbid_ld, int64_t forbid_from,
                      const int64_t* forbid_codes4, int64_t keep_code, int64_t late_forbid_code, int64_t pad_code,
                      const float* finished, int top_k, float top_p, int sample, uint64_t* state, int64_t* out,
                      dvq_stream_t stream);
int dvq_attn_causal_ok(int dtype, int64_t B, int64_t T, int n_head, int head_dim);
int64_t dvq_attn_causal_scratch_bytes(int64_t B, int64_t T, int n_head, int head_dim, int backward);
int64_t dvq_attn_causal_mask_bytes(int64_t B, int64_t T, int n_head);
int dvq_attn_causal_fwd(const void* q, const void* k, const void* v, int64_t ldqkv, int dtype, int64_t B, int64_t T, int n_head,
                        int head_dim, float scale, float p_drop, uint64_t seed, void* out, float* lse, void* scratch, void* drop_mask,
                        dvq_stream_t stream);
int dvq_attn_causal_bwd(const void* q, const void* k, const void* v, int64_t ldqkv, const void* out, const void* dout, const float* lse,
                        int dtype, int64_t B, int64_t T, int n_head, int head_dim, float scale, float p_drop, uint64_t seed, void* dq,
                        void* dk, void* dv, void* scratch, const void* drop_mask, dvq_stream_t stream);
int dvq_attn_full_ok(int dtype, int64_t B, int64_t T, int C);
int dvq_attn_full_fwd(const void* q, const void* k, const void* v, int dtype, int64_t B, int64_t T, int C, float scale, void* out,
                      float* lse, void* scratch, dvq_stream_t stream);
int dvq_attn_full_bwd(const void* q, const void* k, const void* v, const void* out, const void* dout, const float* lse, int dtype,
                      int64_t B, int64_t T, int C, float scale, void* dq, void* dk, void* dv, void* scratch, dvq_stream_t stream);
int dvq_attn_decode(const void* q, const void* kcache, const void* vcache, int dtype, int64_t B, int64_t n_head, int64_t head_size,
                    int64_t T, int64_t Tmax, float scale, void* out, dvq_stream_t stream);
int dvq_attn_decode_dev(const void* q, const void* k_new, const void* v_new, void* kcache, void* vcache, int dtype, int64_t B,
                        int64_t n_head, int64_t head_size, const int64_t* t_dev, int64_t Tmax, float scale, void* out,
                        dvq_stream_t stream);
int dvq_rows_dev(void* x, void* hidden, int dtype, int64_t B, int64_t C, int64_t Tmax, const int64_t* t_dev, int store,
                 dvq_stream_t stream);

typedef struct dvq_decode_layer {
    const void *wq, *wk, *wv, *wo, *w1, *w2;
    const float *bq, *bk, *bv, *bo, *b1, *b2;
    const float *ln1_g, *ln1_b, *ln2_g, *ln2_b;
    void *kcache, *vcache;
} dvq_decode_layer;
size_t dvq_decode_stack_scratch_bytes(int64_t B, int64_t C, int64_t F);
int dvq_decode_stack_ok(int64_t B, int64_t C, int n_head, int64_t F, int64_t Tmax);
int dvq_decode_stack_status(const void* scratch, int64_t B, int64_t C, int64_t F, int reset, dvq_stream_t stream);
int dvq_decode_stack(const void* layers_dev, int n_layers, int64_t B, int64_t C, int n_head, int64_t F, int64_t Tmax, const int64_t* t_dev,
                     float eps, void* x, void* scratch, int n_workgroups, const void* layers_host, dvq_stream_t stream);
int dvq_dropout(const void* x, int dtype, int64_t n, float p, uint64_t seed, void* y, dvq_stream_t stream);
int dvq_dropout_add(const void* x, const void* a, int dtype, int64_t n, float p, uint64_t seed, void* y, dvq_stream_t stream);
int dvq_label_dropout(const int64_t* labels, int64_t B, float p, int64_t null_label, uint64_t seed, int64_t* out, dvq_stream_t stream);

int dvq_adamw_dev(float* p, const float* g, float* m, float* v, int64_t n, const float* hyper, dvq_stream_t stream);
size_t dvq_grad_sqnorm_workspace_bytes(int64_t n);
int dvq_grad_sqnorm(const float* g, int64_t n, float clip, int skip_nonfinite, void* workspace, size_t workspace_bytes,
                    void* gstat, dvq_stream_t stream);
int dvq_adamw_clip_dev(float* p, const float* g, float* m, float* v, int64_t n, const float* hyper, const void* gstat,
                       dvq_stream_t stream);
int dvq_ema_update(float* e, const float* p, int64_t n, const float* rec, const void* gstat, dvq_stream_t stream);
int dvq_swap_f32(float* a, float* b, int64_t n, dvq_stream_t stream);
size_t dvq_segment_stats_workspace_bytes(int64_t n, int64_t S);
size_t dvq_segment_stats_state_bytes(int64_t S);
size_t dvq_segment_plan_bytes(const int64_t* offsets, int64_t S, int64_t n);
int dvq_segment_plan_build(const int64_t* offsets, int64_t S, int64_t n, void* plan_host, size_t plan_host_bytes);
int dvq_segment_stats(const float* a, const float* b, int64_t n, const int64_t* offsets, int64_t S, const void* plan_dev,
                      size_t plan_bytes, void* workspace, size_t workspace_bytes, void* state, int sticky, const int* armed,
                      dvq_stream_t stream);
int dvq_copy_f32_armed(float* dst, const float* src, int64_t n, const int* armed, dvq_stream_t stream);
int dvq_set_f32x8(float* dst, float v0, float v1, float v2, float v3, float v4, float v5, float v6, float v7,
                  dvq_stream_t stream);
enum { DVQ_SCALAR_F32 = 0, DVQ_SCALAR_BF16 = 1, DVQ_SCALAR_F64 = 2, DVQ_SCALAR_I32 = 3, DVQ_SCALAR_I64 = 4, DVQ_SCALAR_IMM = 5,
       DVQ_SCALAR_SKIP = 6  };
enum { DVQ_SCALAR_PUSH_MAX = 64, DVQ_SCALAR_COLUMNS_MAX = 256 };
typedef struct {
    uint64_t addr[64];
    uint8_t code[64];
} dvq_scalar_record;
size_t dvq_scalar_push_state_bytes(int64_t columns);
int dvq_scalar_push(const dvq_scalar_record* rec, int32_t count, int32_t col0, int32_t columns, void* state, dvq_stream_t stream);
int dvq_codebook_health(const void* counts, int counts_type, int64_t K, int64_t stride, float* out3, double* out3_f64, double* total,
                        dvq_stream_t stream);
int dvq_sample_rows(int64_t* out, int64_t k, int64_t n, uint64_t* state, dvq_stream_t stream);
int dvq_add_uniform(float* x, int64_t n, float scale, uint64_t* state, dvq_stream_t stream);

int dvq_fill_f32(float* p, float v, int64_t n, dvq_stream_t stream);

size_t dvq_image_desc_bytes(void);
int dvq_image_batch_transform(const uint8_t* src, const void* desc, const int32_t* tables, uint8_t* tmp, int64_t B, int S,
                              int max_rows, float* out, dvq_stream_t stream);

enum {
    DVQ_JPEG_SUPPORTED = 0,
    DVQ_JPEG_NOT_JPEG = 1,
    DVQ_JPEG_MALFORMED = 2,
    DVQ_JPEG_PROGRESSIVE = 3,
    DVQ_JPEG_ARITHMETIC = 4,
    DVQ_JPEG_SOF_KIND = 5,
    DVQ_JPEG_PRECISION = 6,
    DVQ_JPEG_COMPONENTS = 7,
    DVQ_JPEG_SAMPLING = 8,
    DVQ_JPEG_COLORSPACE = 9,
    DVQ_JPEG_MULTISCAN = 10
};
typedef struct dvq_jpeg_info_t {
    int32_t width, height, components, restart_interval;
    int32_t h_samp[4], v_samp[4], qtab_index[4];
    int32_t supported;
    int32_t reserved;
    int64_t coef_count;
} dvq_jpeg_info_t;
int dvq_jpeg_info(const uint8_t* data, size_t n, dvq_jpeg_info_t* info);
int dvq_jpeg_entropy_decode(const uint8_t* data, size_t n, int16_t* coef, int64_t coef_capacity, uint16_t* qtab);
// ... 63 lines not shown
```

Baseline: 448.1.

## Fuse AttnBlock q/k/v 1x1 convolutions into one packed GEMM with pitched attention

AttnBlock now packs the q, k and v 1x1 conv weights and biases into one concatenated weight, so the forward runs a single 3C-wide convolution instead of three. Attention forward and backward read q/k/v as column slices through a row pitch. The backward produces dq/dk/dv into one strided buffer, runs a single dgrad over the fused weight, and computes per-block wgrads with a new pitched wgrad entry. This is meant to cut kernel launches and repeated reads of the normalized input, at the cost of new pitched pack, wgrad and attention APIs plus fused-pack epoch tracking.

```diff
diff --git a/dynamicvectorquantization_amd/_lib.py b/dynamicvectorquantization_amd/_lib.py
--- a/dynamicvectorquantization_amd/_lib.py
+++ b/dynamicvectorquantization_amd/_lib.py
@@ -31,7 +31,7 @@
 
 class PackEntry(C.Structure):
     _fields_ = [("master", vp), ("w", vp), ("wt", vp), ("Cout", i64), ("Cin", i64), ("taps", i64), ("Cin_p", i64),
-                ("Cout_p", i64), ("begin", i64), ("dtype", i64)]
+                ("Cout_p", i64), ("begin", i64), ("dtype", i64), ("wt_ld", i64), ("bias_src", vp), ("bias_dst", vp)]
 
 
 class ScalarRecord(C.Structure):
@@ -118,6 +118,9 @@
     "dvq_pack_weights_multi": (i32, [vp, i64, i64, vp]),
     "dvq_linear_pack_multi": (i32, [vp, i64, i64, vp]),
     "dvq_pack_weight": (i32, [vp, i64, i64, i64, i64, i64, i64, i32, vp, vp, vp]),
+    "dvq_pack_weight_ld": (i32, [vp, i64, i64, i64, i64, i64, i64, i32, vp, vp, i64, vp, vp, vp]),
+    "dvq_pack_entry_bytes": (i64, []),
+    "dvq_conv2d_wgrad_ld": (i32, [C.POINTER(ConvDesc), vp, vp, i64, i64, i64, vp, vp, i32, vp]),
     "dvq_unpack_wgrad": (i32, [vp, i64, i64, i64, i64, i64, vp, vp]),
     "dvq_nchw_to_nhwc_pad": (i32, [vp, i64, i64, i64, i64, i64, i32, vp, vp]),
     "dvq_nhwc_pad_to_nchw": (i32, [vp, i32, i64, i64, i64, i64, i64, vp, vp]),
@@ -156,6 +159,9 @@
     "dvq_attn_full_ok": (i32, [i32, i64, i64, i32]),
     "dvq_attn_full_fwd": (i32, [vp, vp, vp, i32, i64, i64, i32, f32, vp, vp, vp, vp]),
     "dvq_attn_full_bwd": (i32, [vp, vp, vp, vp, vp, vp, i32, i64, i64, i32, f32, vp, vp, vp, vp, vp]),
+    "dvq_attn_full_ld_ok": (i32, [i32, i64, i64, i32, i64]),
+    "dvq_attn_full_fwd_ld": (i32, [vp, vp, vp, i64, i32, i64, i64, i32, f32, vp, vp, vp, vp]),
+    "dvq_attn_full_bwd_ld": (i32, [vp, vp, vp, i64, vp, vp, vp, i32, i64, i64, i32, f32, vp, vp, vp, vp, vp]),
     "dvq_attn_decode_dev": (i32, [vp, vp, vp, vp, vp, i32, i64, i64, i64, vp, i64, f32, vp, vp]),
     "dvq_rows_dev": (i32, [vp, vp, i32, i64, i64, i64, vp, i32, vp]),
     "dvq_decode_stack_scratch_bytes": (sz, [i64, i64, i64]),
diff --git a/dynamicvectorquantization_amd/csrc/attention.hip b/dynamicvectorquantization_amd/csrc/attention.hip
--- a/dynamicvectorquantization_amd/csrc/attention.hip
+++ b/dynamicvectorquantization_amd/csrc/attention.hip
@@ -474,8 +474,8 @@
         return "%s: bad geometry (T %% 8 == 0, B * n_head <= 65535)";
     if (!((double)B * n_head * (double)T * (double)T < 4294967296.0))
         return "%s: B * n_head * T * T must stay below 2^32 (dropout element index)";
-    if (ld != (int64_t)n_head * head_dim && head_dim != 128)
-        return "%s: a row pitch other than n_head * head_dim needs head size 128 (the kernels of attention2.hip)";
+    if (ld != (int64_t)n_head * head_dim && head_dim == 64)
+        return "%s: a row pitch other than n_head * head_dim needs head size 128 or 256 (the kernels of attention2.hip)";
     if (!(ld >= (int64_t)n_head * head_dim && ld % 8 == 0 && (double)T * (double)ld * 2.0 < 4294967296.0))
         return "%s: bad pitch (at least n_head * head_dim, a multiple of 8, T * pitch * 2 below 2^32)";
     return nullptr;
@@ -506,6 +506,9 @@
     return attn_refusal(dtype, B, T, n_head, head_dim, (int64_t)n_head * head_dim, 0.f, 1) == nullptr;
 }
 int dvq_attn_full_ok(int dtype, int64_t B, int64_t T, int C) { return attn_refusal(dtype, B, T, 1, C, C, 0.f, 0) == nullptr; }
+int dvq_attn_full_ld_ok(int dtype, int64_t B, int64_t T, int C, int64_t ldqkv) {
+    return attn_refusal(dtype, B, T, 1, C, ldqkv, 0.f, 0) == nullptr;
+}
 
 int64_t dvq_attn_causal_scratch_bytes(int64_t B, int64_t T, int n_head, int head_dim, int backward) {
     const int64_t copy = head_dim == 64 ? B * T * n_head * head_dim * 2 : 0;
@@ -574,11 +577,11 @@
     return DVQ_OK;
 }
 
-int dvq_attn_full_fwd(const void* q, const void* k, const void* v, int dtype, int64_t B, int64_t T, int C, float scale, void* out,
-                      float* lse, void* , dvq_stream_t stream) {
+int dvq_attn_full_fwd_ld(const void* q, const void* k, const void* v, int64_t ldqkv, int dtype, int64_t B, int64_t T, int C, float scale,
+                         void* out, float* lse, void* , dvq_stream_t stream) {
     DVQ_REQUIRE(q && k && v && out && lse, DVQ_EINVAL, "dvq_attn_full_fwd: null pointer");
     AttnArgs p{};
-    int rc = fill_params(p, "dvq_attn_full_fwd", dtype, B, T, 1, C, C, scale, 0.f, 0, 0);
+    int rc = fill_params(p, "dvq_attn_full_fwd", dtype, B, T, 1, C, ldqkv, scale, 0.f, 0, 0);
     if (rc != DVQ_OK) return rc;
     p.q = (const bf16_t*)q; p.k = (const bf16_t*)k; p.v = (const bf16_t*)v;
     p.out = (bf16_t*)out; p.lse = lse;
@@ -587,11 +590,17 @@
     return DVQ_OK;
 }
 
-int dvq_attn_full_bwd(const void* q, const void* k, const void* v, const void* out, const void* dout, const float* lse, int dtype,
-                      int64_t B, int64_t T, int C, float scale, void* dq, void* dk, void* dv, void* scratch, dvq_stream_t stream) {
+int dvq_attn_full_fwd(const void* q, const void* k, const void* v, int dtype, int64_t B, int64_t T, int C, float scale, void* out,
+                      float* lse, void* scratch, dvq_stream_t stream) {
+    return dvq_attn_full_fwd_ld(q, k, v, C, dtype, B, T, C, scale, out, lse, scratch, stream);
+}
+
+int dvq_attn_full_bwd_ld(const void* q, const void* k, const void* v, int64_t ldqkv, const void* out, const void* dout, const float* lse,
+                         int dtype, int64_t B, int64_t T, int C, float scale, void* dq, void* dk, void* dv, void* scratch,
+                         dvq_stream_t stream) {
     DVQ_REQUIRE(q && k && v && out && dout && lse && dq && dk && dv && scratch, DVQ_EINVAL, "dvq_attn_full_bwd: null pointer");
     AttnArgs p{};
-    int rc = fill_params(p, "dvq_attn_full_bwd", dtype, B, T, 1, C, C, scale, 0.f, 0, 0);
+    int rc = fill_params(p, "dvq_attn_full_bwd", dtype, B, T, 1, C, ldqkv, scale, 0.f, 0, 0);
     if (rc != DVQ_OK) return rc;
     p.q = (const bf16_t*)q; p.k = (const bf16_t*)k; p.v = (const bf16_t*)v; p.o = (const bf16_t*)out; p.dout = (const bf16_t*)dout;
     p.dq = (bf16_t*)dq; p.dk = (bf16_t*)dk; p.dv = (bf16_t*)dv;
@@ -602,4 +611,9 @@
     return DVQ_OK;
 }
 
-}
+int dvq_attn_full_bwd(const void* q, const void* k, const void* v, const void* out, const void* dout, const float* lse, int dtype,
+                      int64_t B, int64_t T, int C, float scale, void* dq, void* dk, void* dv, void* scratch, dvq_stream_t stream) {
+    return dvq_attn_full_bwd_ld(q, k, v, C, out, dout, lse, dtype, B, T, C, scale, dq, dk, dv, scratch, stream);
+}
+
+}
diff --git a/dynamicvectorquantization_amd/csrc/igemm.hip b/dynamicvectorquantization_amd/csrc/igemm.hip
--- a/dynamicvectorquantization_amd/csrc/igemm.hip
+++ b/dynamicvectorquantization_amd/csrc/igemm.hip
@@ -285,6 +285,20 @@
     DVQ_REQUIRE(gn_scale_shift == nullptr, DVQ_ESHAPE, "dvq_conv2d_wgrad: fused GroupNorm needs a shape accepted by dvq_conv3x3_fused_ok");
     DVQ_REQUIRE(d->impl != DVQ_IMPL_HALO, DVQ_ESHAPE, "dvq_conv2d_wgrad: shape not eligible for the halo kernel");
     const TnParams p = conv_tn_params(d, x, dy, cin_real, cout_real, grad, dbias, ohwi);
+    if (d->dtype == DVQ_F32) return launch_tn<float>(p, 1, d->impl, (hipStream_t)stream);
+    return launch_tn<bf16_t>(p, 1, d->impl, (hipStream_t)stream);
+}
+
+int dvq_conv2d_wgrad_ld(const dvq_conv_desc* d, const void* x, const void* dy, int64_t ldy, int64_t cin_real, int64_t cout_real,
+                        float* grad, float* dbias, int ohwi, dvq_stream_t stream) {
+    if (int e = conv_check(d, "dvq_conv2d_wgrad_ld")) return e;
+    DVQ_REQUIRE(x && dy && grad && cin_real > 0 && cin_real <= d->Cin && cout_real > 0 && cout_real <= d->Cout,
+                DVQ_EINVAL, "dvq_conv2d_wgrad_ld: bad arguments");
+    DVQ_REQUIRE(ldy >= d->Cout && ldy % (d->dtype == DVQ_F32 ? 4 : 8) == 0 && d->N * d->OH * d->OW * ldy < (1ll << 31), DVQ_ESHAPE,
+                "dvq_conv2d_wgrad_ld: bad pitch (at least Cout, a multiple of the vector width, pixels * pitch below 2^31)");
+    DVQ_REQUIRE(!halo_eligible(d) && d->impl != DVQ_IMPL_HALO, DVQ_ESHAPE, "dvq_conv2d_wgrad_ld: the 3x3 halo kernels take no dy pitch");
+    TnParams p = conv_tn_params(d, x, dy, cin_real, cout_real, grad, dbias, ohwi);
+    p.lda = ldy;
     if (d->dtype == DVQ_F32) return launch_tn<float>(p, 1, d->impl, (hipStream_t)stream);
     return launch_tn<bf16_t>(p, 1, d->impl, (hipStream_t)stream);
 }
diff --git a/dynamicvectorquantization_amd/csrc/misc.hip b/dynamicvectorquantization_amd/csrc/misc.hip
--- a/dynamicvectorquantization_amd/csrc/misc.hip
+++ b/dynamicvectorquantization_amd/csrc/misc.hip
@@ -321,10 +321,12 @@
 template <typename T>
 __global__ __launch_bounds__(256) void pack_weight_kernel(const float* __restrict__ m, int64_t Cout, int64_t Cin,
                                                           int64_t KH, int64_t KW, int64_t Cin_p, int64_t Cout_p,
-                                                          T* __restrict__ w, T* __restrict__ wt, bool ohwi, bool sub) {
+                                                          T* __restrict__ w, T* __restrict__ wt, bool ohwi, bool sub, int64_t wt_ld,
+                                                          const float* __restrict__ bias_src, float* __restrict__ bias_dst) {
     const int64_t taps = KH * KW;
     const int64_t nw = w ? Cout * taps * Cin_p : 0, nwt = wt ? Cin * taps * Cout_p : 0, nsub = sub ? 16 * Cout * Cin : 0;
     for (int64_t e = (int64_t)blockIdx.x * 256 + threadIdx.x; e < nw + nwt + 2 * nsub; e += (int64_t)gridDim.x * 256) {
+        if (bias_dst != nullptr && e < Cout) bias_dst[e] = bias_src[e];
         if (e >= nw + nwt) {
             const int64_t f = e - nw - nwt;
             if (f < nsub) ElemIO<T>::store(w + nw + f, subpixel_w_at(m, (unsigned)f, (unsigned)Cout, (unsigned)Cin, ohwi));
@@ -335,7 +337,7 @@
         } else {
             const int64_t f = e - nw;
             const int64_t co = f % Cout_p, tap = (f / Cout_p) % taps, ci = f / (Cout_p * taps);
-            ElemIO<T>::store(wt + f, co < Cout ? master_at(m, co, ci, tap, Cin, taps, ohwi) : 0.f);
+            ElemIO<T>::store(wt + (f / Cout_p) * wt_ld + co, co < Cout ? master_at(m, co, ci, tap, Cin, taps, ohwi) : 0.f);
         }
     }
 }
@@ -347,6 +349,9 @@
     int64_t Cout, Cin, taps, Cin_p, Cout_p;
     int64_t begin;
     int64_t dtype;
+    int64_t wt_ld;
+    const float* bias_src;
+    float* bias_dst;
 };
 
 __device__ __forceinline__ float master_at(const float* m, int64_t co, int64_t ci, int64_t tap, int64_t Cin, int64_t taps, bool ohwi) {
@@ -366,6 +371,11 @@
         const unsigned nw = t.w ? Cout * taps * (unsigned)t.Cin_p : 0u;
         const bool ohwi = (t.dtype >> 8) & 1;
         const unsigned nwt = t.wt ? Cin * taps * (unsigned)t.Cout_p : 0u;
+        if (t.bias_dst != nullptr && f0 < Cout) {
+#pragma unroll
+            for (int u = 0; u < 4; ++u)
+                if (f0 + u < Cout) t.bias_dst[f0 + u] = t.bias_src[f0 + u];
+        }
         float v[4];
         void* dst;
         unsigned di;
@@ -388,7 +398,7 @@
 #pragma unroll
             for (int u = 0; u < 4; ++u) v[u] = co + u < Cout ? master_at(t.master, co + u, ci, tap, Cin, taps, ohwi) : 0.f;
             dst = t.wt;
-            di = f;
+            di = t.wt_ld != 0 ? row * (unsigned)t.wt_ld + co : f;
         }
         if ((t.dtype & 0xff) == DVQ_F32) {
             *reinterpret_cast<float4*>(reinterpret_cast<float*>(dst) + di) = make_float4(v[0], v[1], v[2], v[3]);
@@ -1103,20 +1113,31 @@
     return DVQ_OK;
 }
 
-int dvq_pack_weight(const float* master, int64_t Cout, int64_t Cin, int64_t KH, int64_t KW, int64_t Cin_p,
-                    int64_t Cout_p, int dtype, void* w, void* wt, dvq_stream_t stream) {
+int dvq_pack_weight_ld(const float* master, int64_t Cout, int64_t Cin, int64_t KH, int64_t KW, int64_t Cin_p, int64_t Cout_p, int dtype,
+                       void* w, void* wt, int64_t wt_ld, const float* bias_src, float* bias_dst, dvq_stream_t stream) {
     DVQ_REQUIRE(master && (w || wt) && Cin_p >= Cin && Cout_p >= Cout, DVQ_EINVAL, "dvq_pack_weight: bad arguments");
     const bool ohwi = (dtype >> 8) & 1;
     const bool sub = (dtype >> 9) & 1;
     DVQ_REQUIRE(!sub || (w && wt && KH == 3 && KW == 3 && Cin_p == Cin && Cout_p == Cout && 16 * Cout * Cin < (1ll << 31)), DVQ_EINVAL,
                 "dvq_pack_weight: sub-pixel packs need both outputs, a 3x3 kernel and unpadded channels");
-    const int64_t n = Cout * KH * KW * Cin_p + Cin * KH * KW * Cout_p + (sub ? 32 * Cout * Cin : 0);
+    if (wt_ld == 0) wt_ld = Cout_p;
+    DVQ_REQUIRE(wt_ld >= Cout_p && wt_ld % 4 == 0 && (wt_ld == Cout_p || !sub), DVQ_EINVAL,
+                "dvq_pack_weight: wt_ld must be at least Cout_p and a multiple of 4 (no sub-pixel packs behind a pitched wt)");
+    DVQ_REQUIRE((bias_dst == nullptr) == (bias_src == nullptr), DVQ_EINVAL, "dvq_pack_weight: bias_src and bias_dst go together");
+    const int64_t n = (w ? Cout * KH * KW * Cin_p : 0) + (wt ? Cin * KH * KW * Cout_p : 0) + (sub ? 32 * Cout * Cin : 0);
     dtype &= 0xff;
     DVQ_DISPATCH_DTYPE(dtype, T, pack_weight_kernel<T><<<dim3(nblocks(n, 256)), dim3(256), 0, (hipStream_t)stream>>>(
-                                     master, Cout, Cin, KH, KW, Cin_p, Cout_p, (T*)w, (T*)wt, ohwi, sub););
+                                     master, Cout, Cin, KH, KW, Cin_p, Cout_p, (T*)w, (T*)wt, ohwi, sub, wt_ld, bias_src, bias_dst););
     DVQ_CHECK_LAUNCH("pack_weight");
     return DVQ_OK;
 }
+
+int dvq_pack_weight(const float* master, int64_t Cout, int64_t Cin, int64_t KH, int64_t KW, int64_t Cin_p,
+                    int64_t Cout_p, int dtype, void* w, void* wt, dvq_stream_t stream) {
+    return dvq_pack_weight_ld(master, Cout, Cin, KH, KW, Cin_p, Cout_p, dtype, w, wt, 0, nullptr, nullptr, stream);
+}
+
+int64_t dvq_pack_entry_bytes(void) { return (int64_t)sizeof(PackEntry); }
 
 int dvq_pack_weights_multi(const void* table_dev, int64_t n_entries, int64_t total_work, dvq_stream_t stream) {
     DVQ_REQUIRE(table_dev && n_entries > 0 && n_entries < (1 << 30) && total_work > 0, DVQ_EINVAL, "dvq_pack_weights_multi: bad arguments");
diff --git a/dynamicvectorquantization_amd/kernels.py b/dynamicvectorquantization_amd/kernels.py
--- a/dynamicvectorquantization_amd/kernels.py
+++ b/dynamicvectorquantization_amd/kernels.py
@@ -404,9 +404,13 @@
     return w, wt
 
 
-def pack_weight_into(master, cin_p, cout_p, dtype, w, wt, subpixel=False):
+def pack_weight_into(master, cin_p, cout_p, dtype, w, wt, subpixel=False, wt_ld=0, bias=None, bias_dst=None):
     cout, cin, kh, kw = master.shape
     flag = dt(dtype) | (PACK_OHWI if is_ohwi(master) else 0) | (PACK_SUBPIXEL if subpixel else 0)
+    if wt_ld or bias_dst is not None:
+        check(lib().dvq_pack_weight_ld(_praw(master), cout, cin, kh, kw, cin_p, cout_p, flag, _p(w), _praw(wt), wt_ld, _p(bias),
+                                       _p(bias_dst), _s()), "dvq_pack_weight_ld")
+        return
     check(lib().dvq_pack_weight(_praw(master), cout, cin, kh, kw, cin_p, cout_p, flag, _p(w), _p(wt), _s()),
           "dvq_pack_weight")
 
@@ -557,6 +561,17 @@
                                int(is_ohwi(grad_oihw)), _p(gn_ss), _s()))
 
 
+def conv2d_wgrad_block(d: ConvDesc, x, dy_block, cin_real, cout_real, grad_oihw, db=None):
+    if dy_block.dim() != 2 or dy_block.stride(1) != 1 or dy_block.shape[1] != d.Cout:
+        raise _lib.DvqError("conv2d_wgrad_block: dy must be a [pixels, Cout] column block with unit column stride")
+    fl, nb = _conv_cost(d, x.element_size())
+    ensure_workspace(x.device)
+    _tag(d, "wgrad")
+    _timed_conv(fl, nb, "dvq_conv2d_wgrad_ld", lambda:
+        lib().dvq_conv2d_wgrad_ld(C.byref(d), _p(x), _praw(dy_block), dy_block.stride(0), cin_real, cout_real, _praw(grad_oihw), _p(db),
+                                  int(is_ohwi(grad_oihw)), _s()))
+
+
 def set_deterministic(on: bool):
     check(lib().dvq_set_deterministic(int(bool(on))), "dvq_set_deterministic")
     _det[0] = bool(on)
@@ -999,23 +1014,31 @@
 
 
 def attn_full_fwd(q, k, v, b, t, scale):
+    ld = _attn_pitch(q, k, v)
     c = q.shape[-1]
-    out = torch.empty_like(q)
+    out = torch.empty(q.shape, dtype=q.dtype, device=q.device)
     lse = torch.empty(b, t, dtype=torch.float32, device=q.device)
     scratch = _attn_scratch(q, b, t, 1, False)
     _timed("attn_full_fwd", 4 * b * t * t * c, 4 * q.numel() * q.element_size(), lambda: check(
-        lib().dvq_attn_full_fwd(_p(q), _p(k), _p(v), dt(q), b, t, c, float(scale), _p(out), _p(lse), _p(scratch), _s()),
+        lib().dvq_attn_full_fwd_ld(_praw(q), _praw(k), _praw(v), ld, dt(q), b, t, c, float(scale), _p(out), _p(lse), _p(scratch), _s()),
         "dvq_attn_full_fwd"))
     return out, lse
 
 
-def attn_full_bwd(q, k, v, out, dout, lse, b, t, scale):
+def attn_full_bwd(q, k, v, out, dout, lse, b, t, scale, grads=None):
+    ld = _attn_pitch(q, k, v)
     c = q.shape[-1]
-    dq, dk, dv = torch.empty_like(q), torch.empty_like(q), torch.empty_like(q)
+    if grads is None:
+        if ld != c:
+            raise _lib.DvqError("attn_full_bwd: q, k, v with a row pitch need grads laid out like them")
+        grads = tuple(torch.empty_like(q) for _ in range(3))
+    if _attn_pitch(*grads) != ld or grads[0].shape != q.shape:
+        raise _lib.DvqError("attn_full_bwd: grads must share the shape and row pitch of q, k, v")
+    dq, dk, dv = grads
     scratch = _attn_scratch(q, b, t, 1, True)
     _timed("attn_full_bwd", 10 * b * t * t * c, 8 * q.numel() * q.element_size(), lambda: check(
-        lib().dvq_attn_full_bwd(_p(q), _p(k), _p(v), _p(out), _p(dout), _p(lse), dt(q), b, t, c, float(scale), _p(dq), _p(dk), _p(dv),
-                                _p(scratch), _s()), "dvq_attn_full_bwd"))
+        lib().dvq_attn_full_bwd_ld(_praw(q), _praw(k), _praw(v), ld, _p(out), _p(dout), _p(lse), dt(q), b, t, c, float(scale),
+                                   _praw(dq), _praw(dk), _praw(dv), _p(scratch), _s()), "dvq_attn_full_bwd"))
     return dq, dk, dv
 
 
diff --git a/dynamicvectorquantization_amd/layers.py b/dynamicvectorquantization_amd/layers.py
--- a/dynamicvectorquantization_amd/layers.py
+++ b/dynamicvectorquantization_amd/layers.py
@@ -561,14 +561,35 @@
     def __init__(self):
         self.items = {}
         self.tables = {}
+        self.fused = {}
         self.retired = []
 
     def register(self, mod, dtype):
         import weakref
         key = (dtype, mod.weight.device)
         self.items.setdefault(key, []).append(weakref.ref(mod))
+        self._retire(key)
+
+    def _retire(self, key):
         for k in [k for k in self.tables if k[:2] == key]:
             self.retired.append(self.tables.pop(k))
+
+    def register_fused(self, owner, dtype):
+        import weakref
+        key = (dtype, owner._fused_packs[dtype]["w"].device)
+        refs = self.fused.setdefault(key, [])
+        if not any(r() is owner for r in refs):
+            refs.append(weakref.ref(owner))
+        self._retire(key)
+
+    def _fused_live(self, dtype, device, group):
+        out = []
+        for o in (r() for r in self.fused.get((dtype, device), [])):
+            f = None if o is None else o._fused_packs.get(dtype)
+            if f is not None and f["w"].device == device and all(getattr(m.weight, "_dvq_group", 0) == group for m in f["convs"]) and \
+                    f["masters"] == tuple(m.weight.data_ptr() for m in f["convs"]):
+                out.append(f)
+        return out
 
     def repack(self, dtype, device, group=0):
         import ctypes
@@ -578,12 +599,14 @@
                 getattr(m.weight, "_dvq_group", 0) == group]
         key = (dtype, device, group)
         live = [m for m in mods if m._packs[dtype]["master"] == m.weight.data_ptr() and m._packs[dtype]["w"].device == device]
-        if len(live) < 2:
+        fused = self._fused_live(dtype, device, group)
+        if len(live) + sum(len(f["convs"]) for f in fused) < 2:
             return
-        sig = tuple((m.weight.data_ptr(), m._packs[dtype]["w"].data_ptr(), m.weight.stride()) for m in live)
+        sig = tuple((m.weight.data_ptr(), m._packs[dtype]["w"].data_ptr(), m.weight.stride()) for m in live) + \
+            tuple((f["masters"], f["w"].data_ptr(), tuple(m.bias.data_ptr() for m in f["convs"])) for f in fused)
         tab = self.tables.get(key)
         if tab is None or tab["sig"] != sig:
-            arr = (PackEntry * len(live))()
+            arr = (PackEntry * (len(live) + sum(len(f["convs"]) for f in fused)))()
             begin = 0
             for i, m in enumerate(live):
                 e = m._packs[dtype]
@@ -594,14 +617,26 @@
                 begin += m.out_channels * k2 * e["cin_p"] + m.in_channels * k2 * e["cout_p"]
                 if e["sub"]:
                     begin += 32 * m.out_channels * m.in_channels
+            i = len(live)
+            es = torch.empty(0, dtype=dtype).element_size()
+            for f in fused:
+                n = len(f["convs"])
+                for j, m in enumerate(f["convs"]):
+                    co, ci = m.out_channels, m.in_channels
+                    arr[i] = PackEntry(m.weight.data_ptr(), f["w"].data_ptr() + j * co * ci * es, f["wt"].data_ptr() + j * co * es,
+                                       co, ci, 1, ci, co, begin, K.dt(dtype), n * co, m.bias.data_ptr(), f["b"].data_ptr() + j * co * 4)
+                    begin += 2 * co * ci
+                    i += 1
             raw = torch.frombuffer(bytearray(bytes(arr)), dtype=torch.uint8).to(device)
-            tab = {"sig": sig, "table": raw, "n": len(live), "total": begin}
+            tab = {"sig": sig, "table": raw, "n": len(arr), "total": begin}
             if key in self.tables:
                 self.retired.append(self.tables[key])
             self.tables[key] = tab
         K.pack_weights_multi(tab["table"], tab["n"], tab["total"])
         for m in live:
             m._packs[dtype]["epoch"] = m._pack_key()
+        for f in fused:
+            f["epoch"] = tuple(m._pack_key() for m in f["convs"])
 
 
 PACKS = _PackRegistry()
@@ -721,11 +756,81 @@
         self.k = Conv2d(in_channels, in_channels, 1)
         self.v = Conv2d(in_channels, in_channels, 1)
         self.proj_out = Conv2d(in_channels, in_channels, 1)
+        self._fused_packs = {}
+
+    def _qkv_pack(self, dtype):
+        convs = (self.q, self.k, self.v)
+        dev = self.q.weight.device
+        masters = tuple(m.weight.data_ptr() for m in convs)
+        ent = self._fused_packs.get(dtype)
+        if ent is None or ent["w"].device != dev or ent["masters"] != masters:
+            c = self.in_channels
+            ent = {"convs": convs, "masters": masters, "epoch": None, "w": torch.zeros(3 * c, 1, 1, c, dtype=dtype, device=dev),
+                   "wt": torch.zeros(c, 1, 1, 3 * c, dtype=dtype, device=dev), "b": torch.zeros(3 * c, dtype=torch.float32, device=dev)}
+            self._fused_packs[dtype] = ent
+            PACKS.register_fused(self, dtype)
+        key = tuple(m._pack_key() for m in convs)
+        if ent["epoch"] != key:
+            if ent["epoch"] is not None:
+                PACKS.repack(dtype, dev, getattr(self.q.weight, "_dvq_group", 0))
+            if ent["epoch"] != key:
+                c = self.in_channels
+                for i, m in enumerate(convs):
+                    K.pack_weight_into(m.weight.detach(), c, c, dtype, ent["w"][i * c:(i + 1) * c], ent["wt"].view(-1)[i * c:],
+                                       wt_ld=3 * c, bias=m.bias.detach(), bias_dst=ent["b"][i * c:(i + 1) * c])
+                ent["epoch"] = key
+        return ent
+
+    def _qkv_fusable(self, x2d, t):
+        c = self.in_channels
+        return (x2d.dtype == torch.bfloat16 and rt.impl() == 0 and rt.switch("DVQ_QKV_FUSED") != "0" and c % 8 == 0 and
+                K.attn_full_ok(x2d, t) and all(m.bias is not None for m in (self.q, self.k, self.v)) and
+                bool(K.lib().dvq_attn_full_ld_ok(K.dt(x2d), x2d.shape[0] // max(1, t), t, c, 3 * c)))
+
+    def _fwd_qkv(self, x, hn, tape):
+        b, h, w, c = x.shape
+        n = h * w
+        pk = self._qkv_pack(hn.dtype)
+        d = K.conv_desc(b, h, w, c, 3 * c, 1, 1, 1, 0, 0, h, w, False, hn.dtype, 0)
+        qkv = K.conv2d_fwd(d, hn, pk["w"], pk["b"]).view(b * n, 3 * c)
+        q, k, v = qkv[:, :c], qkv[:, c:2 * c], qkv[:, 2 * c:]
+        o, lse = K.attn_full_fwd(q, k, v, b, n, float(int(c) ** (-0.5)))
+        y = self.proj_out.fwd(o.view(b, h, w, c), _child(tape, "proj"), residual=x)
+        if tape is not None:
+            tape.s.update(qkv=qkv, hn=hn, o=o, lse=lse, p=None, shape=(b, h, w, c))
+        return y
+
+    def _bwd_qkv(self, dy, tape):
+        st = tape.s
+        b, h, w, c = st["shape"]
+        n = h * w
+        qkv, hn = st["qkv"], st["hn"]
+        do = self.proj_out.bwd(dy, tape.child("proj"))
+        dqkv = torch.empty_like(qkv)
+        (q, k, v), (dq, dk, dv) = (tuple(m_[:, i * c:(i + 1) * c] for i in range(3)) for m_ in (qkv, dqkv))
+        K.attn_full_bwd(q, k, v, st["o"], do.view(b * n, c), st["lse"], b, n, float(int(c) ** (-0.5)), grads=(dq, dk, dv))
+        pk = self._qkv_pack(qkv.dtype)
+        d3 = K.conv_desc(b, h, w, c, 3 * c, 1, 1, 1, 0, 0, h, w, False, qkv.dtype, 0)
+        d1 = K.conv_desc(b, h, w, c, c, 1, 1, 1, 0, 0, h, w, False, qkv.dtype, 0)
+        dh = K.conv2d_dgrad(d3, dqkv.view(b, h, w, 3 * c), pk["wt"])
+        grads = [(_grad_buf(m.weight), _grad_buf(m.bias)) for m in (self.q, self.k, self.v)]
+
+        def wgrad():
+            for (gw, gb), blk in zip(grads, (dq, dk, dv)):
+                K.conv2d_wgrad_block(d1, hn, blk, c, c, gw, gb)
+
+        if rt.side_wgrad_enabled():
+            rt.run_on_side(wgrad, hn, dqkv)
+        else:
+            wgrad()
+        return self.norm.bwd(dh, tape.child("norm"), addend=dy)
 
     def fwd(self, x, tape):
         b, h, w, c = x.shape
         n = h * w
         hn = self.norm.fwd(x, _child(tape, "norm"), silu=False)
+        if self._qkv_fusable(hn.view(b * n, c), n):
+            return self._fwd_qkv(x, hn, tape)
         q = self.q.fwd(hn, _child(tape, "q"))
         k = self.k.fwd(hn, _child(tape, "k"))
         v = self.v.fwd(hn, _child(tape, "v"))
@@ -748,6 +853,8 @@
 
     def bwd(self, dy, tape):
         st = tape.s
+        if "qkv" in st:
+            return self._bwd_qkv(dy, tape)
         b, h, w, c = st["shape"]
         n = h * w
         q, k, v, p = st["q"], st["k"], st["v"], st["p"]
diff --git a/dynamicvectorquantization_amd/runtime.py b/dynamicvectorquantization_amd/runtime.py
--- a/dynamicvectorquantization_amd/runtime.py
+++ b/dynamicvectorquantization_amd/runtime.py
@@ -19,7 +19,7 @@
     "DVQ_X3_WGRAD_PLANES": ("1", "0: fp32x3 weight gradients on the fp32 kernel that splits at every fragment read"),
     "DVQ_NO_FUSED_ATTN": ("0", "1: causal attention as per-head GEMMs + softmax instead of the fused kernels"),
     "DVQ_NO_FUSED_ATTNBLOCK": ("0", "1: AttnBlock on GEMMs + softmax (stores the [B,N,N] probabilities)"),
-    "DVQ_QKV_FUSED": ("1", "0: key / query / value as three Linear layers instead of one GEMM"),
+    "DVQ_QKV_FUSED": ("1", "0: key / query / value as three Linear layers (StackGPT) / 1x1 convolutions (AttnBlock) instead of one GEMM"),
     "DVQ_FUSE_DROP_BWD": ("1", "0: stand-alone dropout passes in the StackGPT backward"),
     "DVQ_GEN_SIDE": ("1", "0: generator loss with the PatchGAN branch on the main stream"),
     "DVQ_LOSS_PREFETCH": ("1", "0: target-only loss work inside the loss call instead of beside the autoencoder's forward"),
diff --git a/include/dvq_hip.h b/include/dvq_hip.h
--- a/include/dvq_hip.h
+++ b/include/dvq_hip.h
@@ -117,12 +117,17 @@
 
 int dvq_conv2d_wgrad(const dvq_conv_desc* d, const void* x, const void* dy, int64_t cin_real, int64_t cout_real, float* grad,
                      float* dbias, int ohwi, const float* gn_scale_shift, dvq_stream_t stream);
+int dvq_conv2d_wgrad_ld(const dvq_conv_desc* d, const void* x, const void* dy, int64_t ldy, int64_t cin_real, int64_t cout_real,
+                        float* grad, float* dbias, int ohwi, dvq_stream_t stream);
 
 int dvq_pack_weights_multi(const void* table_dev, int64_t n_entries, int64_t total_work, dvq_stream_t stream);
 int dvq_linear_pack_multi(const void* table_dev, int64_t n_entries, int64_t total_tiles, dvq_stream_t stream);
 
 int dvq_pack_weight(const float* master, int64_t Cout, int64_t Cin, int64_t KH, int64_t KW, int64_t Cin_p,
                     int64_t Cout_p, int dtype, void* w, void* wt, dvq_stream_t stream);
+int dvq_pack_weight_ld(const float* master, int64_t Cout, int64_t Cin, int64_t KH, int64_t KW, int64_t Cin_p, int64_t Cout_p, int dtype,
+                       void* w, void* wt, int64_t wt_ld, const float* bias_src, float* bias_dst, dvq_stream_t stream);
+int64_t dvq_pack_entry_bytes(void);
 int dvq_unpack_wgrad(const float* dw, int64_t Cout, int64_t Cin, int64_t KH, int64_t KW, int64_t Cin_p, float* grad,
                      dvq_stream_t stream);
 int dvq_nchw_to_nhwc_pad(const float* in, int64_t B, int64_t C, int64_t H, int64_t W, int64_t Cp, int dtype, void* out,
@@ -245,6 +250,12 @@
                       float* lse, void* scratch, dvq_stream_t stream);
 int dvq_attn_full_bwd(const void* q, const void* k, const void* v, const void* out, const void* dout, const float* lse, int dtype,
                       int64_t B, int64_t T, int C, float scale, void* dq, void* dk, void* dv, void* scratch, dvq_stream_t stream);
+int dvq_attn_full_ld_ok(int dtype, int64_t B, int64_t T, int C, int64_t ldqkv);
+int dvq_attn_full_fwd_ld(const void* q, const void* k, const void* v, int64_t ldqkv, int dtype, int64_t B, int64_t T, int C, float scale,
+                         void* out, float* lse, void* scratch, dvq_stream_t stream);
+int dvq_attn_full_bwd_ld(const void* q, const void* k, const void* v, int64_t ldqkv, const void* out, const void* dout, const float* lse,
+                         int dtype, int64_t B, int64_t T, int C, float scale, void* dq, void* dk, void* dv, void* scratch,
+                         dvq_stream_t stream);
 int dvq_attn_decode(const void* q, const void* kcache, const void* vcache, int dtype, int64_t B, int64_t n_head, int64_t head_size,
                     int64_t T, int64_t Tmax, float scale, void* out, dvq_stream_t stream);
 int dvq_attn_decode_dev(const void* q, const void* k_new, const void* v_new, void* kcache, void* vcache, int dtype, int64_t B,
```

New measurement: 449.0 (median of 6 runs). Within noise of the previous version (+0.2%).
